# NeuroDiffGym/neurodiffeq

Hardware: AMD Instinct MI355X
Metric: collocation-points/sec (residual+bwd), 2D Laplace 65k pts, 1/2/4/8 GPU (higher is better)
Workload: dtype f32; 1 GPU; C2: Solver2D 2D Laplace, DirichletBVP2D, FCNN(2-32-32-1, tanh), Generator2D 256x256 = 65536 noisy-grid points per GPU per step, Adam(1e-3), run_train_epoch() with n_batches_train=1, n_batches_valid=0; points_per_gpu=65536, global_batch=65536, parallelism=dp1 (shard-by-batch, one all-reduce of [P+1] fp32 per step), allreduce=none (single process), inputs=pre-sampled in the reference's RNG order, resident in HBM

## Files before the change

__graft_entry__.py:

```python
import os
import sys

ROOT = os.path.dirname(os.path.abspath(__file__))
if ROOT not in sys.path:
    sys.path.insert(0, ROOT)


def build():
    from neurodiffeq_amd import _hipcc
    with _hipcc.deferred():
        built = _build_all()
    from neurodiffeq_amd import codegen
    for f in ([] if os.environ.get("NDQ_BUILD_NO_PRUNE") else os.listdir(codegen.JIT_DIR)):
        path = os.path.join(codegen.JIT_DIR, f)
        if path not in built and os.path.splitext(path)[0] + ".so" not in built:
            if os.path.isdir(path):
                import shutil
                shutil.rmtree(path, ignore_errors=True)
            else:
                os.remove(path)
    missing = [b for b in built if not os.path.exists(b)]
    assert not missing, f"build() did not produce {missing}"


# ... 34 lines not shown
        systems.append((name, nets, conds, pde, z.n_coords, None))
    pde, conds = zoo.spherical_solver_problem()
    systems.append(("spherical-default", [FCNN(3, 1)], conds, pde, 3, None))
    from neurodiffeq_amd import diff
    from neurodiffeq_amd.conditions import IVP
    losses = {}
    for name, kind in (("helmholtz_xy", "l1"), ("stokes_like", "l1"), ("stokes_like", "infinity"), ("pendulum", "infinity")):
        z = zoo.build(name)
        nets, conds, pde = z.product()
        systems.append((f"{name}/{kind}", nets, conds, pde, z.n_coords, None))
        losses[f"{name}/{kind}"] = kind
    systems.append(("default-ode/l1", [FCNN(1, 1)], [IVP(0.0, 1.0)], lambda u, t: [diff(u, t) + u], 1, None))
    losses["default-ode/l1"] = "l1"
    systems.append(("default-ode", [FCNN(1, 1)], [IVP(0.0, 1.0)], lambda u, t: [diff(u, t) + u], 1, None))
    from neurodiffeq_amd.solvers import sobolev_equations
    lv = lambda u, v, t: [diff(u, t) - (u - u * v), diff(v, t) - (u * v - v)]
    for semi in (False, True):
        systems.append((f"lotka-volterra/h1{' semi' if semi else ''}", [FCNN(1, 1), FCNN(1, 1)], [IVP(0.0, 1.5), IVP(0.0, 1.0)],
                        sobolev_equations(lv, 2, semi), 1, None))
    from neurodiffeq_amd.conditions import NoCondition
    systems.append(("helmholtz/h1", [FCNN(2, 1)], [NoCondition()],
                    sobolev_equations(lambda u, x, y: [diff(u, x, order=2) + diff(u, y, order=2) - u], 1, False), 2, None))
    for name in ("shell", "poisson3d", "hessian3d", "pendulum", "shape_48x2", "shape_32x3"):
        z = zoo.build(name)
        nets, conds, pde = z.product()
        systems.append((f"{name}/group", nets, conds, pde, z.n_coords, None))
    import warnings
    shared = FCNN(1, 2, hidden_units=(32, 32))
    sconds = [IVP(0.0, 1.5), IVP(0.0, 1.0)]
    with warnings.catch_warnings():
        warnings.simplefilter("ignore")
        sconds[0].set_impose_on(0)
        sconds[1].set_impose_on(1)
    systems.append(("shared-net", [shared, shared], sconds, lv, 1, None))
    from functools import partial
    from neurodiffeq_amd.networks import Resnet, Swish
    c4 = configs.make("c4", 8)
    systems.append(("c4/resnet", [Resnet(1, 25, hidden_units=(32, 32))], c4["conds"], configs.fused_equations(c4),
                    configs.n_coords(c4), configs.func_val(c4)))
    c2 = configs.make("c2", 8)
    systems.append(("c2/swish-trainable", [FCNN(2, 1, hidden_units=(32, 32), actv=partial(Swish, trainable=True))], c2["conds"],
                    configs.fused_equations(c2), configs.n_coords(c2), configs.func_val(c2)))
    c2n, c3n = configs.make("c2", 8), configs.make("c3", 8)
    systems.append(("c2/nolap", c2n["nets"], c2n["conds"], configs.fused_equations(c2n), 2, None))
    systems.append(("c2/columns", c2n["nets"], c2n["conds"],
                    lambda u, x, y: [diff(u, x), diff(u, y), diff(u, x, order=2), diff(u, y, order=2)], 2, None))
    systems.append(("c3/columns", c3n["nets"], c3n["conds"],
                    lambda u, x, y: [diff(u, x), diff(u, y), diff(u, x, order=2)], 2, None))
    for name in ("inv1", "inv2"):
        torch.manual_seed(0)
        icfg = configs.make_inverse(name)
        systems.append((name, icfg["nets"], icfg["conds"], icfg["pde"], 2 if name == "inv1" else 1, None))
    from tests import sampler_table_problems
    for axes in (2, 4):
        torch.manual_seed(0)
        tcfg = sampler_table_problems.bundle_problem(axes)
        systems.append((f"table-bundle-{axes}", tcfg["nets"], tcfg["conds"], tcfg["pde"], axes, None))
    csolver, ccfg = configs.make_custom_loss_solver(16)
    systems.append(("custom-loss", ccfg["nets"], ccfg["conds"], ccfg["pde"], 2, None))
    losses["custom-loss"] = lambda r, f, x: csolver.loss_fn(r, f, x) + csolver.additional_loss(r, f, x)
    metrics = {"custom-loss": list(csolver.metrics_fn.values())}
    for name, nets, conds, pde, nc, cfv in systems:
        os.environ.pop("NDQ_FUSE_GROUP", None)
        os.environ.pop("NDQ_NO_LAP", None)
        if name.endswith("/group"):
            os.environ["NDQ_FUSE_GROUP"] = "1"
        if name.endswith("/nolap"):
            os.environ["NDQ_NO_LAP"] = "1"
        program, descs = trace_system(nets, conds, pde, nc, compute_func_val=cfv, loss=losses.get(name, "l2"),
                                      metrics=metrics.get(name, ()))
        so = codegen.build(program)
        built.add(so)
        print("built", so, f"({name}: {len(program.symbols)} stream symbols, {len(program.order)} nodes)", flush=True)
        if codegen.can_fuse(program, descs):
            so = codegen.build_fused(program, descs[0])
            built.add(so)
            print("built", so, f"({name}: single-launch fused closure, {len(nets)} network(s))", flush=True)
            if name in ("c2", "pendulum", "advection", "helmholtz_xy", "sigmoid_mixed") and codegen.fuse_mode(program, descs) == "tile":
                so = codegen.build_fused(program, descs[0], threads=512)
                built.add(so)
                print("built", so, f"({name}: 8-wave build of the closure kernel)", flush=True)
    os.environ.pop("NDQ_FUSE_GROUP", None)
    os.environ.pop("NDQ_NO_LAP", None)
    f64_systems = []
    for name, size in (("c1", 8), ("c2", 8), ("c3", 8)):
        torch.manual_seed(0)
        cfg = configs.make(name, size)
        if name == "c3":
            cfg["nets"] = [FCNN(2, 1, hidden_units=(32, 32, 32))]
        f64_systems.append((name, cfg["nets"], cfg["conds"], configs.fused_equations(cfg), configs.n_coords(cfg), configs.func_val(cfg)))
    for name in ("pendulum", "helmholtz_xy", "stokes_like", "sigmoid_mixed", "kdv", "resnet_laplace", "swish_tr_laplace",
                 "aptx_tr_resnet", "shape_20x3", "mono_ode", "ensemble_lv", "shape_48x2", "shape_64x2"):
        z = zoo.build(name)
        nets, conds, pde = z.product()
        f64_systems.append((name, nets, conds, pde, z.n_coords, None))
    for name in ("c1", "c2", "c4", "w1", "w2", "w3", "w4", "w5", "w6", "w7", "w8", "w9", "w10", "w11", "w12", "w13", "w14", "w15",
                 "w16", "w17"):
        torch.manual_seed(0)
        cfg = configs.make(name, {"c1": 64, "c2": 16, "c4": 96}.get(name))
        f64_systems.append((name + "/golden", cfg["nets"], cfg["conds"], configs.fused_equations(cfg), configs.n_coords(cfg),
                            configs.func_val(cfg)))
    for name, nets, conds, pde, nc, cfv in f64_systems:
        for net in nets:
            net.double()
        program, descs = trace_system(nets, conds, pde, nc, compute_func_val=cfv, f64=True)
        so = codegen.build(program, f64=True)
        built.add(so)
        print("built", so, f"({name}: fp64 pointwise kernel)", flush=True)
        if codegen.can_fuse_f64(program, descs):
            so = codegen.build_fused(program, descs[0], f64=True)
            built.add(so)
            print("built", so, f"({name}: fp64 single-launch closure)", flush=True)
    from neurodiffeq_amd import autograd_ops
    for name in ("c1", "c2", "c3", "c4", "c5"):
        for net in configs.make(name, 8)["nets"][:1]:
            for order in (0, 1, 2):
                assert autograd_ops._spec_for(net, order) is not None, (name, order)
    for net in (FCNN(3, 2, hidden_units=(32, 32)), FCNN(1, 1), FCNN(3, 1)):
        for order in (0, 2):
            assert autograd_ops._spec_for(net, order) is not None
    for net in (FCNN(1, 1), FCNN(2, 1)):
        assert autograd_ops._spec_for(net, 3) is not None
    for L64 in (_lib.lib64(),):
        for sym in _lib.EXPORTS64:
            getattr(L64, sym)
    for d, act, n_out, order in ((2, 0, 3, 1), (3, 0, 1, 2), (1, 2, 1, 3), (2, 1, 1, 0), (1, 0, 1, 0), (2, 0, 1, 0)):
        assert codegen.ensure_mlp_kernels(autograd_ops._desc(d, order, 32, 2, act, n_out), f64=True), (d, act, n_out, order)
    for args in ((1, 1, 1, 32, 2, 1, 1, 0, 0, 1), (2, 1, 7, 32, 2, 0, 1, 0, 0, 15), (2, 1, 1, 32, 2, 0, 1, 0, 0, 1),
                 (2, 1, 5, 64, 3, 0, 1, 0, 0, 9), (1, 1, 1, 32, 2, 2, 2, 0, 0, 1), (3, 1, 22, 32, 2, 0, 1, 0, 0, 16)):
        assert codegen.ensure_mlp_kernels(_lib.MlpDesc(*args)), args
    assert codegen.ensure_mlp_kernels(autograd_ops._desc(2, 4, 32, 2, 0, 1)), "order-4 stream set of the autograd seam"
    from tests import test_gpu_parity as gp
    gp.ARCH.update(gp.ARCH_T4)
    try:
        for name in gp.ARCH_T4:
            assert codegen.ensure_mlp_kernels(gp._desc(name)), name
    finally:
        for name in gp.ARCH_T4:
            gp.ARCH.pop(name, None)
    from tests import test_gpu_netfamily as nf
    from tests import test_gpu_wide as wd
    ext_descs = [nf._desc(name) for name in nf.CASES]
    for shape in wd.SHAPES:
        ext_descs.append(wd.shape_desc(shape)[0])
    with _hipcc.deferred():
        for desc in ext_descs:
            if not L.ndq_mlp_supported(ctypes.byref(desc)) and codegen.mlp_ext_allowed(desc):
                codegen.build_mlp_ext(desc)
    for name in nf.CASES:
        assert codegen.ensure_mlp_kernels(nf._desc(name)), name
    from tests import test_gpu_wide as wd
    for shape in wd.SHAPES:
        assert codegen.ensure_mlp_kernels(wd.shape_desc(shape)[0]), shape
    built |= {ext._name for ext in codegen._MLP_EXT.values() if ext is not None}
    if os.path.isdir("/root/reference/neurodiffeq"):
        subprocess.run(["bash", os.path.join(ROOT, "oracle", "make_ref.sh")], check=True)
    return built


def smoke():
    import numpy as np
    import torch
    from oracle import autograd_ref as R
    from tests import configs
    assert torch.cuda.is_available(), "smoke() needs cuda:0"
    torch.cuda.set_device(0)
# ... 24 lines not shown
```

include/ndq.h:

```cpp
#ifndef NDQ_H
#define NDQ_H
#include <stddef.h>
#ifdef __cplusplus
extern "C" {
#endif

#define NDQ_EUNSUPPORTED (-1)
#define NDQ_EINVAL (-2)

#define NDQ_ACT_TANH 0
#define NDQ_ACT_SIN 1
#define NDQ_ACT_SIGMOID 2
#define NDQ_ACT_SWISH 3
#define NDQ_ACT_APTX 4
#define NDQ_ACT_ELU 5
#define NDQ_ACT_SOFTPLUS 6
#define NDQ_ACT_GELU 7

#define NDQ_MAX_HIDDEN 512
typedef struct ndq_mlp_desc {
  int d;
  int first;
  int mask2;
  int hidden;
// ... 44 lines not shown
                   float beta2, float eps, float weight_decay, int step, const float* loss_slots, int n_batches,
                   float* loss_hist, int hist_index, float* best_loss, int parity, float* best_flat, int write_scalars,
                   void* stream);

#define NDQ_SAMPLE_UNIFORM 0
#define NDQ_SAMPLE_GRID 1
#define NDQ_SAMPLE_SPHERICAL 2
typedef struct ndq_sampler_desc {
  int kind;
  int d;
  int n[3];
  float lo[3], hi[3];
  float noise_std[3];
  int radial;
} ndq_sampler_desc;
int ndq_sample(const ndq_sampler_desc* desc, unsigned long long seed, unsigned long long draw, unsigned stream_id,
               float* coords, int ldc, void* stream);

#define NDQ_TABLE_MAX_AXES 6
#define NDQ_AXIS_NORMAL 0
#define NDQ_AXIS_CHEB2_NOISY 1
typedef struct ndq_table_sampler_desc {
  int d;
  int n[NDQ_TABLE_MAX_AXES];
  int law[NDQ_TABLE_MAX_AXES];
  int abs_value;
  const float* mean[NDQ_TABLE_MAX_AXES];
  const float* std[NDQ_TABLE_MAX_AXES];
  float lo[NDQ_TABLE_MAX_AXES], hi[NDQ_TABLE_MAX_AXES];
} ndq_table_sampler_desc;
int ndq_sample_table(const ndq_table_sampler_desc* desc, unsigned long long seed, unsigned long long draw,
                     unsigned stream_id, float* coords , int ldc, void* stream);

#define NDQ_PLAN_MAX_LEAVES 8
#define NDQ_LEAF_SIMPLE 0
#define NDQ_LEAF_TABLE 1
#define NDQ_LEAF_DATA 2
#define NDQ_SEG_LEAF 0
#define NDQ_SEG_ENSEMBLE 1
#define NDQ_SEG_MESH 2
typedef struct ndq_plan_leaf {
  int kind;
  int row0;
  int rows;
  int n;
  union {
    ndq_sampler_desc simple;
    ndq_table_sampler_desc table;
    const float* data[NDQ_TABLE_MAX_AXES];
  } u;
} ndq_plan_leaf;
typedef struct ndq_plan_segment {
  int mode;
  int first, count;
  int offset, size;
} ndq_plan_segment;
typedef struct ndq_plan_sampler_desc {
  int d;
  int n_leaves;
  int n_segments;
  int reserved;
  ndq_plan_leaf leaf[NDQ_PLAN_MAX_LEAVES];
  ndq_plan_segment seg[NDQ_PLAN_MAX_LEAVES];
} ndq_plan_sampler_desc;
int ndq_sample_plan(const ndq_plan_sampler_desc* desc, unsigned long long seed, unsigned long long draw,
                    unsigned stream_id, float* coords , int ldc, void* stream);

#define NDQ_INDEX_NONE 0
#define NDQ_INDEX_PERMUTE 1
#define NDQ_INDEX_REPLACE 2
typedef struct ndq_plan_index_desc {
  int mode;
  int m;
  int batch;
  int reserved;
} ndq_plan_index_desc;
int ndq_sample_plan_indexed(const ndq_plan_sampler_desc* desc, const ndq_plan_index_desc* index, unsigned long long seed,
                            unsigned long long draw, unsigned stream_id, float* coords , int ldc, void* stream);

typedef int (*ndq_fused_launch_fn)(const float* coords, int ldc, int n, const float* params, float* partials,
                                   float* loss_partials, float* funcs, float* resid, int ldj, float seed, int train,
                                   void* stream);

typedef int (*ndq_allreduce_fn)(const void* sendbuf, void* recvbuf, size_t count, int dtype, int op, void* comm,
                                void* stream);

typedef struct ndq_fused_step {
  ndq_fused_launch_fn launch;
  int n, ldc, ldj, blocks, n_params;
  float seed;
  float* params;
  float* partials;
  float* loss_partials;
  float* grad;
  float* loss_slot;
  float* adam_m;
  float* adam_v;
  float lr, beta1, beta2, eps, weight_decay;
  float* loss_hist;
  float* best_loss;
  float* best_flat;
  ndq_allreduce_fn allreduce;
  void* comm;
  const struct ndq_sampler_desc* next_sampler;
  unsigned long long next_seed, next_draw;
  unsigned next_stream;
  float* next_coords;
  int next_ldc;
} ndq_fused_step;
int ndq_fused_step_run(const ndq_fused_step* s, const float* coords, int adam_step, int hist_index, int parity,
                       void* stream);

typedef int (*ndq_fused_launch_multi_fn)(const float* coords, int ldc, int n, const float* const* params,
                                         float* const* partials, float* loss_partials, float* funcs, float* resid,
                                         int ldj, float seed, int train, void* stream);
int ndq_fused_multi_step_run(const ndq_fused_step* steps, int n_nets, ndq_fused_launch_multi_fn launch,
                             const float* coords, int adam_step, int hist_index, int parity, void* stream);

typedef int (*ndq_fused_launch_tv_fn)(const float* coords, int ldc, int n, const float* const* params,
                                      float* const* partials, float* loss_partials, float seed,
                                      const float* valid_coords, int valid_ldc, int valid_n,
                                      float* valid_loss_partials, const void* pull, void* stream);
typedef int (*ndq_fused_launch_loop_fn)(const float* coords, int ldc, int n, float seed, const float* vcoords, int vldc,
                                        int vn, const void* loop, void* stream);
typedef struct ndq_fused_fit {
  ndq_fused_launch_tv_fn launch;
  int n_nets;
  ndq_fused_step net[4];
  const float* valid_coords;
  int valid_n, valid_ldc, valid_blocks;
  float valid_scale;
  float* valid_loss_partials;
  float* valid_hist;
  int track_best;
  int pull_ok;
  float* alt_params[4];
  float* alt_m[4];
  float* alt_v[4];
  float* alt_partials[4];
  float* alt_loss_partials;
  float* alt_valid_loss_partials;
  ndq_fused_launch_loop_fn launch_loop;
  int loop_ok;
} ndq_fused_fit;
int ndq_fused_fit_run(const ndq_fused_fit* f, int n_epochs, const float* const* train_coords, int adam_step,
                      int hist_index, int valid_index, int parity, void* stream);

typedef int (*ndq_pointwise_fn)(const float* coords, int ldc, int n, const float* const* jets,
                                float* const* gbar, int ldj, float* funcs, float* resid, float* loss_partials,
                                float seed_scale, void* stream);
typedef int (*ndq_pw_blocks_fn)(int n);
typedef void (*ndq_bind_theta_fn)(const float* theta, float* theta_partials);

typedef struct ndq64_mlp_kernels {
  ndq_mlp_desc desc;
  int n_streams, n_params;
  int bwd_waves;
  int lds_bytes;
  int (*fwd)(const double* coords, int ldc, int n, const double* params, double* jets, int ldj, void* stream);
  int (*bwd)(const double* coords, int ldc, int n, const double* params, const double* gbar, int ldj, double* partials,
             int blocks, void* stream);
} ndq64_mlp_kernels;
int ndq64_mlp_register(const ndq64_mlp_kernels* kernels);
int ndq64_mlp_supported(const ndq_mlp_desc* desc);
int ndq64_mlp_num_streams(const ndq_mlp_desc* desc);
int ndq64_mlp_num_params(const ndq_mlp_desc* desc);
int ndq64_mlp_bwd_blocks(const ndq_mlp_desc* desc, int n);
int ndq64_mlp_jet_fwd(const ndq_mlp_desc* desc, const double* coords, int ldc, int n, const double* params, double* jets,
                      int ldj, void* stream);
int ndq64_mlp_jet_bwd(const ndq_mlp_desc* desc, const double* coords, int ldc, int n, const double* params,
                      const double* gbar, int ldj, double* partials, void* stream);
int ndq64_reduce_partials(const double* partials, int nparts, int len, double* out, int accumulate, double scale,
                          void* stream);
int ndq64_adam_step(double* params, const double* grad, double* exp_avg, double* exp_avg_sq, int len, double lr,
                    double beta1, double beta2, double eps, double weight_decay, int step, void* stream);

int ndq64_epoch_tail(double* params, const double* grad, double* exp_avg, double* exp_avg_sq, int len, double lr,
                     double beta1, double beta2, double eps, double weight_decay, int step, const double* loss_slots,
                     int n_batches, double* loss_hist, int hist_index, double* best_loss, int parity, double* best_flat,
                     int write_scalars, void* stream);

int ndq_oneshot_create(int rank, int world_size, int max_len, void** ctx, unsigned char* handle64);
int ndq_oneshot_connect(void* ctx, const unsigned char* handles);
int ndq_oneshot_allreduce(const void* send, void* recv, size_t count, int dtype, int op, void* ctx, void* stream);
int ndq_oneshot_status(void* ctx);
int ndq_oneshot_destroy(void* ctx);

#ifdef __cplusplus
}
#endif
#endif
// ... 1 lines not shown
```

neurodiffeq_amd/_lib.py:

```python
import ctypes
import os

from . import _build

NDQ_ACT_TANH, NDQ_ACT_SIN, NDQ_ACT_SIGMOID, NDQ_ACT_SWISH, NDQ_ACT_APTX = 0, 1, 2, 3, 4
NDQ_ACT_ELU, NDQ_ACT_SOFTPLUS, NDQ_ACT_GELU = 5, 6, 7


class MlpDesc(ctypes.Structure):
    _fields_ = [("d", ctypes.c_int), ("first", ctypes.c_int), ("mask2", ctypes.c_int), ("hidden", ctypes.c_int),
                ("layers", ctypes.c_int), ("act", ctypes.c_int), ("n_out", ctypes.c_int), ("lap", ctypes.c_int),
                ("skip", ctypes.c_int), ("mask3", ctypes.c_int), ("actp", ctypes.c_int), ("widths", ctypes.c_int), ("mono", ctypes.c_int),
                ("mask4", ctypes.c_int)]

    def key(self):
        return (self.d, self.first, self.mask2, self.hidden, self.layers, self.act, self.n_out, self.lap, self.skip,
                self.mask3, self.actp, self.widths, self.mono, self.mask4)


NDQ_SAMPLE_UNIFORM, NDQ_SAMPLE_GRID, NDQ_SAMPLE_SPHERICAL = 0, 1, 2


class SamplerDesc(ctypes.Structure):
    _fields_ = [("kind", ctypes.c_int), ("d", ctypes.c_int), ("n", ctypes.c_int * 3), ("lo", ctypes.c_float * 3),
                ("hi", ctypes.c_float * 3), ("noise_std", ctypes.c_float * 3), ("radial", ctypes.c_int)]


NDQ_TABLE_MAX_AXES = 6
NDQ_AXIS_NORMAL, NDQ_AXIS_CHEB2_NOISY = 0, 1


class TableSamplerDesc(ctypes.Structure):
    _fields_ = [("d", ctypes.c_int), ("n", ctypes.c_int * 6), ("law", ctypes.c_int * 6), ("abs_value", ctypes.c_int),
                ("mean", ctypes.c_void_p * 6), ("std", ctypes.c_void_p * 6), ("lo", ctypes.c_float * 6),
                ("hi", ctypes.c_float * 6)]


NDQ_PLAN_MAX_LEAVES = 8
NDQ_LEAF_SIMPLE, NDQ_LEAF_TABLE, NDQ_LEAF_DATA = 0, 1, 2
NDQ_SEG_LEAF, NDQ_SEG_ENSEMBLE, NDQ_SEG_MESH = 0, 1, 2
NDQ_INDEX_NONE, NDQ_INDEX_PERMUTE, NDQ_INDEX_REPLACE = 0, 1, 2


class _PlanLaw(ctypes.Union):
    _fields_ = [("simple", SamplerDesc), ("table", TableSamplerDesc), ("data", ctypes.c_void_p * 6)]


class PlanLeaf(ctypes.Structure):
    _fields_ = [("kind", ctypes.c_int), ("row0", ctypes.c_int), ("rows", ctypes.c_int), ("n", ctypes.c_int), ("u", _PlanLaw)]


class PlanSegment(ctypes.Structure):
    _fields_ = [("mode", ctypes.c_int), ("first", ctypes.c_int), ("count", ctypes.c_int), ("offset", ctypes.c_int),
                ("size", ctypes.c_int)]


class PlanSamplerDesc(ctypes.Structure):
    _fields_ = [("d", ctypes.c_int), ("n_leaves", ctypes.c_int), ("n_segments", ctypes.c_int), ("reserved", ctypes.c_int),
                ("leaf", PlanLeaf * 8), ("seg", PlanSegment * 8)]


class PlanIndexDesc(ctypes.Structure):
    _fields_ = [("mode", ctypes.c_int), ("m", ctypes.c_int), ("batch", ctypes.c_int), ("reserved", ctypes.c_int)]


FUSED_LAUNCH_FN = ctypes.CFUNCTYPE(ctypes.c_int, ctypes.c_void_p, ctypes.c_int, ctypes.c_int, ctypes.c_void_p,
                                   ctypes.c_void_p, ctypes.c_void_p, ctypes.c_void_p, ctypes.c_void_p, ctypes.c_int,
                                   ctypes.c_float, ctypes.c_int, ctypes.c_void_p)


class FusedStep(ctypes.Structure):
    _fields_ = [("launch", ctypes.c_void_p),
                ("n", ctypes.c_int), ("ldc", ctypes.c_int), ("ldj", ctypes.c_int), ("blocks", ctypes.c_int),
                ("n_params", ctypes.c_int), ("seed", ctypes.c_float),
                ("params", ctypes.c_void_p), ("partials", ctypes.c_void_p), ("loss_partials", ctypes.c_void_p),
                ("grad", ctypes.c_void_p), ("loss_slot", ctypes.c_void_p), ("adam_m", ctypes.c_void_p),
                ("adam_v", ctypes.c_void_p),
                ("lr", ctypes.c_float), ("beta1", ctypes.c_float), ("beta2", ctypes.c_float), ("eps", ctypes.c_float),
                ("weight_decay", ctypes.c_float),
                ("loss_hist", ctypes.c_void_p), ("best_loss", ctypes.c_void_p), ("best_flat", ctypes.c_void_p),
                ("allreduce", ctypes.c_void_p), ("comm", ctypes.c_void_p),
                ("next_sampler", ctypes.c_void_p), ("next_seed", ctypes.c_ulonglong), ("next_draw", ctypes.c_ulonglong),
                ("next_stream", ctypes.c_uint), ("next_coords", ctypes.c_void_p), ("next_ldc", ctypes.c_int)]


class FusedFit(ctypes.Structure):
    _fields_ = [("launch", ctypes.c_void_p), ("n_nets", ctypes.c_int), ("net", FusedStep * 4),
                ("valid_coords", ctypes.c_void_p), ("valid_n", ctypes.c_int), ("valid_ldc", ctypes.c_int),
                ("valid_blocks", ctypes.c_int), ("valid_scale", ctypes.c_float),
                ("valid_loss_partials", ctypes.c_void_p), ("valid_hist", ctypes.c_void_p), ("track_best", ctypes.c_int),
                ("pull_ok", ctypes.c_int), ("alt_params", ctypes.c_void_p * 4), ("alt_m", ctypes.c_void_p * 4),
                ("alt_v", ctypes.c_void_p * 4), ("alt_partials", ctypes.c_void_p * 4),
                ("alt_loss_partials", ctypes.c_void_p), ("alt_valid_loss_partials", ctypes.c_void_p),
                ("launch_loop", ctypes.c_void_p), ("loop_ok", ctypes.c_int)]


class NdqError(RuntimeError):
    pass


_LIB = None


def lib():
    global _LIB
    if _LIB is not None:
        return _LIB
    path = _build.LIB
    if _build.is_stale():
        try:
            _build.build_lib()
        except Exception as e:
            if not os.path.exists(path):
                raise NdqError(f"libndq.so is missing and could not be built: {e}") from e
    L = ctypes.CDLL(path)
    vp, ci, cf = ctypes.c_void_p, ctypes.c_int, ctypes.c_float
    dp = ctypes.POINTER(MlpDesc)
    L.ndq_mlp_supported.argtypes = [dp]
    L.ndq_mlp_num_streams.argtypes = [dp]
    L.ndq_mlp_num_params.argtypes = [dp]
    L.ndq_mlp_bwd_blocks.argtypes = [dp, ci]
    L.ndq_mlp_jet_fwd.argtypes = [dp, vp, ci, ci, vp, vp, ci, vp]
    L.ndq_mlp_jet_bwd.argtypes = [dp, vp, ci, ci, vp, vp, ci, vp, vp]
    L.ndq_reduce_partials.argtypes = [vp, ci, ci, vp, ci, cf, vp]
    L.ndq_adam_step.argtypes = [vp, vp, vp, vp, ci, cf, cf, cf, cf, cf, ci, vp]
    L.ndq_reduce_grad_loss.argtypes = [vp, ci, ci, vp, ci, vp, ci, vp, cf, vp]
    L.ndq_epoch_tail.argtypes = [vp, vp, vp, vp, ci, cf, cf, cf, cf, cf, ci, vp, ci, vp, ci, vp, ci, vp, ci, vp]
    L.ndq_fused_step_run.argtypes = [ctypes.POINTER(FusedStep), vp, ci, ci, ci, vp]
    L.ndq_fused_multi_step_run.argtypes = [ctypes.POINTER(FusedStep), ci, vp, vp, ci, ci, ci, vp]
    L.ndq_fused_fit_run.argtypes = [ctypes.POINTER(FusedFit), ci, vp, ci, ci, ci, ci, vp]
    L.ndq_mlp_register.argtypes = [vp]
    L.ndq_sample.argtypes = [ctypes.POINTER(SamplerDesc), ctypes.c_ulonglong, ctypes.c_ulonglong, ctypes.c_uint, vp, ci, vp]
    L.ndq_sample_table.argtypes = [ctypes.POINTER(TableSamplerDesc), ctypes.c_ulonglong, ctypes.c_ulonglong, ctypes.c_uint, vp, ci,
                                   vp]
    L.ndq_sample_plan.argtypes = [ctypes.POINTER(PlanSamplerDesc), ctypes.c_ulonglong, ctypes.c_ulonglong, ctypes.c_uint, vp, ci, vp]
    L.ndq_sample_plan_indexed.argtypes = [ctypes.POINTER(PlanSamplerDesc), ctypes.POINTER(PlanIndexDesc), ctypes.c_ulonglong,
                                          ctypes.c_ulonglong, ctypes.c_uint, vp, ci, vp]
    L.ndq_oneshot_create.argtypes = [ci, ci, ci, ctypes.POINTER(vp), ctypes.c_char_p]
    L.ndq_oneshot_connect.argtypes = [vp, ctypes.c_char_p]
    L.ndq_oneshot_allreduce.argtypes = [vp, vp, ctypes.c_size_t, ci, ci, vp, vp]
    L.ndq_oneshot_status.argtypes = [vp]
    L.ndq_oneshot_destroy.argtypes = [vp]
    for name in ("ndq_mlp_supported", "ndq_mlp_num_streams", "ndq_mlp_num_params", "ndq_mlp_bwd_blocks",
                 "ndq_mlp_jet_fwd", "ndq_mlp_jet_bwd", "ndq_reduce_partials", "ndq_adam_step", "ndq_reduce_grad_loss",
                 "ndq_epoch_tail", "ndq_fused_step_run", "ndq_sample", "ndq_sample_table", "ndq_sample_plan", "ndq_sample_plan_indexed", "ndq_mlp_register",
                 "ndq_fused_multi_step_run", "ndq_fused_fit_run", "ndq_oneshot_create", "ndq_oneshot_connect",
                 "ndq_oneshot_allreduce", "ndq_oneshot_status",
                 "ndq_oneshot_destroy"):
        getattr(L, name).restype = ci
    _LIB = L
    return L


_LIB64 = None


def lib64():
    global _LIB64
    if _LIB64 is not None:
        return _LIB64
    if _build.is_stale64():
        try:
            _build.build_lib64()
        except Exception as e:
            if not os.path.exists(_build.LIB64):
                raise NdqError(f"libndq64.so is missing and could not be built: {e}") from e
# ... 35 lines not shown
```

neurodiffeq_amd/codegen.py:

```python
import ctypes
import hashlib
import os
import re

from .symbolic import Graph, TraceUnsupported

HERE = os.path.dirname(os.path.abspath(__file__))
JIT_DIR = os.path.join(HERE, "_jit")
from . import _hipcc


def _extra_flags():
    return os.environ.get("NDQ_JIT_FLAGS", "").split()


def pair_list(d):
    return [(a, b) for a in range(d) for b in range(a, d)]


def triple_list(d):
    return [(a, b, c) for a in range(d) for b in range(a, d) for c in range(b, d)]


CLOSURE_PRODUCTS = ("#ifndef NDQ_HBAR_NPROD\n#define NDQ_HBAR_NPROD 4\n#endif\n"
# ... 34 lines not shown
            self.mask2 |= 1 << pair_list(self.d).index(loc)
        if len(loc) == 3:
            self.mask3 |= 1 << triple_list(self.d).index(loc)
            for pair in ((loc[0], loc[1]), (loc[0], loc[2]), (loc[1], loc[2])):
                self.mask2 |= 1 << pair_list(self.d).index(pair)
        if len(loc) == 4:
            if self.d > 3:
                raise TraceUnsupported("fourth-order derivatives of a network with more than three inputs are outside the fused path")
            self.mask4 |= 1 << quad_list(self.d).index(loc)
            for i in range(4):
                tri = tuple(loc[j] for j in range(4) if j != i)
                self.mask3 |= 1 << triple_list(self.d).index(tri)
                for j in range(i + 1, 4):
                    self.mask2 |= 1 << pair_list(self.d).index((loc[i], loc[j]))
        if len(loc) > 4:
            raise TraceUnsupported("derivatives of network outputs beyond fourth order are outside the fused path")

    @property
    def n_streams(self):
        return (1 + self.first * self.d + (1 if self.lap else bin(self.mask2).count("1")) + bin(self.mask3).count("1")
                + bin(self.mask4).count("1"))

    def slot(self, mi):
        if mi and mi[0] == "L":
            return 1 + self.d
        assert not (self.lap and len(mi) == 2)
        loc = tuple(sorted(self.deps.index(c) for c in mi))
        if len(loc) == 0:
            return 0
        if len(loc) == 1:
            return 1 + loc[0]
        if len(loc) == 4:
            k = quad_list(self.d).index(loc)
            assert (self.mask4 >> k) & 1 and not self.lap
            return 1 + self.d + bin(self.mask2).count("1") + bin(self.mask3).count("1") + bin(self.mask4 & ((1 << k) - 1)).count("1")
        if len(loc) == 3:
            k = triple_list(self.d).index(loc)
            assert (self.mask3 >> k) & 1 and not self.lap
            return 1 + self.d + bin(self.mask2).count("1") + bin(self.mask3 & ((1 << k) - 1)).count("1")
        k = pair_list(self.d).index(loc)
        assert (self.mask2 >> k) & 1
        return 1 + self.d + bin(self.mask2 & ((1 << k) - 1)).count("1")


def _lit(v):
    if v != v or v in (float("inf"), float("-inf")):
        raise ValueError("non-finite constant in traced expression")
    s = repr(float(v))
    if "." not in s and "e" not in s and "n" not in s:
        s += ".0"
    return s + "f"


def _powi_expr(x, n):
    if n == 0:
        return "1.0f"
    if n == 1:
        return x
    if n <= 8:
        return "(" + "*".join([x] * n) + ")"
    return f"powf({x}, {float(n)}f)"


_UN_FWD = {
    "neg": "-{a}", "sin": "sinf({a})", "cos": "cosf({a})", "tan": "tanf({a})", "exp": "expf({a})",
    "log": "logf({a})", "tanh": "tanhf({a})", "sqrt": "sqrtf({a})", "abs": "fabsf({a})", "sinh": "sinhf({a})",
    "cosh": "coshf({a})", "sigmoid": "(1.0f/(1.0f+expf(-{a})))", "recip": "(1.0f/{a})",
    "sign": "(({a}>0.0f)-({a}<0.0f))",
    "log1p": "log1pf({a})", "expm1": "expm1f({a})", "erf": "erff({a})", "atan": "atanf({a})",
    "floor": "floorf({a})", "ceil": "ceilf({a})", "round": "rintf({a})", "trunc": "truncf({a})",
    "detach": "{a}",
}
_UN_ADJ = {
    "neg": "-{b}", "sin": "{b}*cosf({a})", "cos": "-{b}*sinf({a})", "tan": "{b}*(1.0f+{v}*{v})",
    "exp": "{b}*{v}", "log": "{b}/{a}", "tanh": "{b}*(1.0f-{v}*{v})", "sqrt": "{b}/(2.0f*{v})",
    "abs": "{b}*(({a}>0.0f)-({a}<0.0f))", "sinh": "{b}*coshf({a})", "cosh": "{b}*sinhf({a})",
    "sigmoid": "{b}*{v}*(1.0f-{v})", "recip": "-{b}*{v}*{v}", "sign": None,
    "log1p": "{b}/(1.0f+{a})", "expm1": "{b}*({v}+1.0f)", "erf": "{b}*1.1283791670955126f*expf(-{a}*{a})",
    "atan": "{b}/(1.0f+{a}*{a})",
    "floor": None, "ceil": None, "round": None, "trunc": None, "detach": None,
}


def _closure_host(K, threads, points, slots, kern, kern_tv, lds, kern_loop=None, lds_loop=None):
    return f"""struct Closure {{
  using Cfg = CFG;
  using Pw = PW;
  using Args = ndq::{'FusedArgs' if K == 1 else 'FusedMultiArgs'};
  static constexpr int K = {K}, THREADS = {threads}, POINTS = {points}, SLOTS = {slots};
  static constexpr auto train = &{kern('true')};
  static constexpr auto eval = &{kern('false')};
  static constexpr auto tv = &{kern_tv};
  static constexpr auto loop = {'&' + kern_loop if kern_loop else 'nullptr'};
  static constexpr size_t LDS_TRAIN = {lds('true')}, LDS_EVAL = {lds('false')}, LDS_LOOP = {lds_loop or 0};
}};
}}  // namespace
#include "ndq_closure_host.h"
"""


class PointwiseProgram:

    LOSS_KINDS = ("l2", "l1", "infinity", "custom")

    def __init__(self, graph: Graph, residuals, funcs, n_nets, widen=None, allow_lap=None, unify=None, loss="l2",
                 loss_term=None):
        assert loss in self.LOSS_KINDS and (loss == "custom") == (loss_term is not None)
        self.loss = loss
        self.g = graph
        self.residuals = list(residuals)
        self.funcs = list(funcs)
        self.loss_term = loss_term
        if allow_lap is not None:
            extra = [loss_term] if loss_term is not None else []
            merged = self._merge_laplacian(self.residuals + extra, self.funcs, n_nets, allow_lap)
            self.residuals = merged[:len(self.residuals)]
            if extra:
                self.loss_term = merged[-1]
        self.n_nets = n_nets
        self.site_net = list(getattr(graph, "site_net", None) or range(n_nets))
        self.n_sites = len(self.site_net)
        self.n_coords = graph.n_coords
        self.n_data = len(getattr(graph, "data", ()))
        self.n_theta = len(getattr(graph, "params", ()))
        self.order = graph.reachable(self.residuals + self.funcs + ([self.loss_term] if self.loss_term is not None else []))
        self.streams = {}
        for k in range(self.n_sites):
            deps = graph.net_deps.get(k)
            if deps is None:
                continue
            self.streams[k] = NetStreams(deps, graph.net_nout[k])
        self.symbols = []
        for i in self.order:
            n = graph.nodes[i]
            if n[0] == "net":
                self.streams[n[1]].need(n[3])
                self.symbols.append(i)
        if unify is not None:
            unify(self.streams)
        if widen is not None:
            for k, st in self.streams.items():
                widen(k, st)
        self.source = self._emit()
        self.key = hashlib.sha1((self.source + _build_tag()).encode()).hexdigest()[:16]

    def _merge_laplacian(self, residuals, funcs, n_nets, allow_lap):
        g = self.g
        order = g.reachable(list(residuals) + list(funcs))
        second = {}
        third = set()
        for i in order:
            n = g.nodes[i]
            if n[0] == "net" and len(n[3]) == 2 and n[3][0] != "L":
                second.setdefault(n[1], []).append(i)
            if n[0] == "net" and len(n[3]) >= 3 and n[3][0] != "L":
                third.add(n[1])
        for k in third:
            second.pop(k, None)
        func_set = set(g.reachable(list(funcs)))
        out = list(residuals)
        for k, leaves in second.items():
            mis = [g.nodes[i][3] for i in leaves]
            if any(a != b for a, b in mis) or len(leaves) < 2:
                continue
            if any(i in func_set for i in leaves):
                continue
            by_out = {}
            for i in leaves:
                by_out.setdefault(g.nodes[i][2], []).append(i)
            coords = sorted({mi[0] for mi in mis})
            if any(sorted(g.nodes[i][3][0] for i in ls) != coords for ls in by_out.values()):
                continue
            leafset = set(leaves)
            ok = True
            for r in out:
                for o, ls in by_out.items():
                    ds = [g.diff(r, ("n", i)) for i in ls]
# ... 136 lines not shown
            i = g._ids.get(("param", j))
            L.append(f"  g[{nsym + j}] = {'b%d' % i if (i is not None and i in terms and i in res_set) else '0.0f'};")
        return "\n".join(L)

    def point_fn_source(self):
        nc = self.n_coords
        body = self._emit_point_fn()
        neq = len(self.residuals)
        if self.loss == "custom":
            term = f"r[{neq}]"
        elif self.loss == "l2":
            term = " + ".join(f"r[{e}]*r[{e}]" for e in range(neq)) or "0.0f"
        elif self.loss == "l1":
            term = " + ".join(f"fabsf(r[{e}])" for e in range(neq)) or "0.0f"
        else:
            term = "0.0f"
            for e in range(neq):
                term = f"fmaxf({term}, fabsf(r[{e}]))"
        nd, nt = self.n_data, self.n_theta
        return f"""// c: {nc} coordinate(s) | {nd} per-point data value(s) | {nt} trainable scalar(s) of the equations;  g: adjoints of the
// {len(self.symbols)} stream symbol(s) | of the {nt} trainable scalar(s)
NDQ_PW_INLINE void ndq_pw_point(const float* c, const float* s, float seed, int want_adj, float* r, float* f, float* g) {{
{chr(10).join(f"  const float c{i} = c[{i}];" for i in range(nc))}
{chr(10).join(f"  const float d{j} = c[{nc + j}];" for j in range(nd))}
{chr(10).join(f"  const float t{j} = c[{nc + nd + j}];" for j in range(nt))}
{chr(10).join(f"  const float c{i} = {_lit(v)};   // virtual coordinate (boundary value)" for i, v in sorted(self.g.vcoords.items()))}
{body}
}}
// per-point loss term ({self.loss}); the host averages it: seed = 1 / (N * n_eq) for l2 / l1, 1 / N for infinity
NDQ_PW_INLINE float ndq_pw_loss(const float* r) {{ return {term}; }}
"""

    @property
    def loss_norm(self):
        return 1 if self.loss in ("infinity", "custom") else max(len(self.residuals), 1)

    @property
    def n_r(self):
        return max(len(self.residuals) + (1 if self.loss == "custom" else 0), 1)

    def fused_source(self, desc, f64=False):
        if f64:
            return "#define NDQ_F64 1\n" + source_f64(self._fused_source(desc, True))
        return self._fused_source(desc, False)

    def _fused_source(self, desc, f64):
        K = self.n_nets
        mode = fuse_mode(self, {k: desc for k in range(K)})
        assert mode is not None and not (f64 and (mode != "tile" or K != 1))
        if mode in ("group", "wide"):
            return self._group_source(desc, wide=(mode == "wide"))
        ns = self.streams[0].n_streams
        nsym = max(len(self.symbols), 1)
        jet = (lambda k, loc: f"jets[{loc}]") if K == 1 else (lambda k, loc: f"jets[{k}][{loc}]")
        gj = (lambda k, loc: f"gj[{loc}]") if K == 1 else (lambda k, loc: f"gj[{k}][{loc}]")
        loads, stores = [], []
        used = {}
        for idx, i in enumerate(self.symbols):
            k, loc = self.sym_location(i)
            used[(k, loc)] = idx
            loads.append(f"    s[{idx}] = {jet(k, loc)};")
        for k in range(K):
            for loc in range(ns):
                stores.append(f"    {gj(k, loc)} = {'g[%d]' % used[(k, loc)] if (k, loc) in used else '0.0f'};")
        header = "ndq_mlp.h"
        neq, nf = len(self.residuals), len(self.funcs)
        jets_t = "const float (&jets)[CFG::NS]" if K == 1 else f"const float (&jets)[{K}][CFG::NS]"
        gj_t = "float (&gj)[CFG::NS]" if K == 1 else f"float (&gj)[{K}][CFG::NS]"
        kern = (lambda train: f"ndq::fused_closure_kernel<CFG, PW, {train}>") if K == 1 else \
            (lambda train: f"ndq::fused_multi_closure_kernel<CFG, {K}, PW, {train}>")
        lds = (lambda train: f"ndq::fused_lds_bytes<CFG>({train})") if K == 1 else \
            (lambda train: f"(ndq::fused_multi_lds_bytes<CFG, {K}>({train}))")
        threads = "CFG::BWD_THREADS" if K == 1 else f"ndq::multi_threads<{K}>()"
        tiles_per_block = "CFG::BWD_THREADS / 64" if K == 1 else f"ndq::multi_group<{K}>()"
        kern_tv = "ndq::fused_closure_tv_kernel<CFG, PW>" if K == 1 else f"ndq::fused_multi_closure_tv_kernel<CFG, {K}, PW>"
        if f64:
            kern_loop = lds_loop = None
        elif K == 1:
            kern_loop, lds_loop = "ndq::fused_closure_loop_kernel<CFG, PW>", "ndq::fused_loop_lds_bytes<CFG>()"
        elif K == 2:
            kern_loop, lds_loop = f"ndq::fused_multi_closure_loop_kernel<CFG, {K}, PW>", f"(ndq::fused_multi_loop_lds_bytes<CFG, {K}>())"
        else:
            kern_loop = lds_loop = None
        host = _closure_host(K, threads, 16, tiles_per_block, kern, kern_tv, lds, kern_loop, lds_loop)
        wg_tr = f"#ifndef NDQ_WG_TR\n#define NDQ_WG_TR 1\n#endif\n#define NDQ_WG_TR_K {K}\n" + CLOSURE_PRODUCTS
        return f"""// GENERATED by neurodiffeq_amd/codegen.py -- single-launch closure kernel (forward streams + pointwise stage +
// reverse pass) of one PDE system with {K} network(s), gfx950.
{wg_tr}#include "{header}"
#define NDQ_PW_INLINE __device__ __forceinline__
#ifndef NDQ_MAX_BLOCKS
#define NDQ_MAX_BLOCKS 256     // closure workgroups per launch (one per CU; experiments: 512 = two 8-wave workgroups per CU)
#endif
{self.point_fn_source()}
namespace {{
using CFG = {mlp_cfg(desc, 1)};
struct PW {{
  // ND per-point data columns (rows D .. D + ND of the coordinate block), NT trainable scalars of the equations
  static constexpr int NEQ = {neq}, NF = {nf}, NR = {self.n_r}, ND = {self.n_data}, NT = {self.n_theta};
  static __device__ __forceinline__ float loss(const float* r) {{ return ndq_pw_loss(r); }}
  // xe: the point's ND data values, then the NT scalars;  gth (want_adj): per-point adjoints of the scalars
  static __device__ __forceinline__ void apply(const float (&x)[CFG::D], const float* xe, {jets_t}, float seed,
                                               int want_adj, float (&r)[{self.n_r}], float (&f)[{max(nf, 1)}],
                                               {gj_t}, float* gth) {{
    float c[CFG::D + ND + NT], s[{nsym}], g[{nsym} + NT];
#pragma unroll
    for (int d = 0; d < CFG::D; ++d) c[d] = x[d];
#pragma unroll
    for (int j = 0; j < ND + NT; ++j) c[CFG::D + j] = xe[j];
{chr(10).join(loads)}
    ndq_pw_point(c, s, seed, want_adj, r, f, g);
{chr(10).join(stores)}
#pragma unroll
    for (int j = 0; j < NT; ++j) gth[j] = g[{len(self.symbols)} + j];
  }}
}};
{host}"""

    def _group_source(self, desc, wide=False):
        st = self.streams[0]
        width = st.n_streams * st.n_out
        gw = 1 if st.n_out == 1 else (st.n_out + 15) // 16 * 16
        if wide:
            gw = st.n_out
        row = lambda loc: (loc // st.n_out) * gw + loc % st.n_out
        nsym = max(len(self.symbols), 1)
        used = {}
        loads = []
        for idx, i in enumerate(self.symbols):
            k, loc = self.sym_location(i)
            used[loc] = idx
            loads.append(f"    s[{idx}] = srow[{row(loc)}];")
        stores = [f"    grow[{row(loc)}] = {'g[%d]' % used[loc] if loc in used else '0.0f'};" for loc in range(width)]
        deps = list(st.deps)
        dep_fn = " : ".join(f"d == {d} ? {c}" for d, c in enumerate(deps)) + " : 0"
        header = "ndq_mlp.h"
        neq, nf = len(self.residuals), len(self.funcs)
        kern = lambda train: f"ndq::fused_group_closure_kernel<CFG, PW, {train}>"
        lds = lambda train: f"ndq::group_lds_bytes<CFG>({train})"
        kern_tv = "ndq::fused_group_closure_tv_kernel<CFG, PW>"
        cfg_t, points = mlp_cfg(desc, desc.n_out), "16 * ndq::group_tiles<CFG>()"
        if wide:
            header = "ndq_wide.h"
            kern = lambda train: f"ndq::wide_closure_kernel<CFG, PW, {train}>"
            lds = lambda train: "(ndq::wide_closure_lds_bytes<CFG, PW>())"
            kern_tv = "ndq::wide_closure_tv_kernel<CFG, PW>"
            cfg_t, points = wide_cfg(desc), 16
        host = _closure_host(1, "CFG::BWD_THREADS", points, "CFG::BWD_THREADS / 64", kern, kern_tv, lds)
        return f"""// GENERATED by neurodiffeq_amd/codegen.py -- grouped single-launch closure kernel (forward streams -> LDS exchange ->
// per-point stage, one point per lane -> reverse pass) of one PDE system, gfx950.
{CLOSURE_PRODUCTS}#include "{header}"
#define NDQ_PW_INLINE __device__ __forceinline__
#ifndef NDQ_MAX_BLOCKS
#define NDQ_MAX_BLOCKS 256     // closure workgroups per launch (one per CU; experiments: 512 = two 8-wave workgroups per CU)
#endif
{self.point_fn_source()}
namespace {{
using CFG = {cfg_t};
static_assert(CFG::NS * CFG::NOUT == {width}, "stream layout of the traced program and of the kernel disagree");
struct PW {{
  // NC rows of the coordinate block per point: the batch coordinates, then ND data columns; NT trainable scalars
  static constexpr int NEQ = {neq}, NF = {nf}, ND = {self.n_data}, NT = {self.n_theta}, NC = {self.n_coords} + ND, NR = {self.n_r};
  static constexpr int dep(int d) {{ return {dep_fn}; }}     // batch coordinate fed to network input d
  static __device__ __forceinline__ float loss(const float* r) {{ return ndq_pw_loss(r); }}
  static __device__ __forceinline__ void apply(const float (&cc)[NC], const float* th, const float* srow, float seed, int want_adj,
                                               float (&r)[{self.n_r}], float (&f)[{max(nf, 1)}], float* grow, float* gth) {{
    float c[NC + NT], s[{nsym}], g[{nsym} + NT];
#pragma unroll
# ... 132 lines not shown
    a.jets[k] = jets[k];
    a.gbar[k] = gbar ? gbar[k] : nullptr;
  }}
  a.funcs = funcs; a.resid = resid; a.loss_partials = loss_partials;
  a.n = n; a.ldc = ldc; a.ldj = ldj; a.want_adj = gbar ? 1 : 0; a.seed = seed_scale;
  hipLaunchKernelGGL(ndq_pw_kernel, dim3((n + 255) / 256), dim3(256), 0, static_cast<hipStream_t>(stream), a);
  return (int)hipGetLastError();
}}
#endif
"""
        return src

    def bytes_per_point(self, train=True, write_resid=False, write_funcs=False):
        b = 4 * self.n_coords + 4 * len(self.symbols)
        if train:
            b += 4 * sum(st.n_streams * st.n_out for st in self.streams.values())
        if write_resid:
            b += 4 * len(self.residuals)
        if write_funcs:
            b += 4 * len(self.funcs)
        return b


class PointwiseKernel:
    def __init__(self, so_path, f64=False):
        self.path = so_path
        self.lib = ctypes.CDLL(so_path)
        self.lib.ndq_pw_launch.restype = ctypes.c_int
        self.lib.ndq_pw_launch.argtypes = [ctypes.c_void_p, ctypes.c_int, ctypes.c_int, ctypes.c_void_p, ctypes.c_void_p,
                                           ctypes.c_int, ctypes.c_void_p, ctypes.c_void_p, ctypes.c_void_p,
                                           ctypes.c_double if f64 else ctypes.c_float, ctypes.c_void_p]
        self.lib.ndq_pw_blocks.restype = ctypes.c_int
        self.lib.ndq_pw_blocks.argtypes = [ctypes.c_int]

    def blocks(self, n):
        return self.lib.ndq_pw_blocks(n)


def so_path_for(program: PointwiseProgram, f64=False):
    return os.path.join(JIT_DIR, f"pw{'64' if f64 else ''}_{program.key}.so")


_F64_FUNCS = re.compile(r"\b(pow|sin|cos|tan|exp|log|tanh|sqrt|fabs|sinh|cosh|fmax|log1p|expm1|erf|atan|atan2|floor|ceil|rint|trunc)f\(")
_F64_LITERAL = re.compile(r"(?<![\w.])((?:\d+\.\d*|\.\d+|\d+)(?:[eE][-+]?\d+)?)f\b")


def source_f64(source):
    out = re.sub(r"\bfloat\b", "double", source)
    out = _F64_FUNCS.sub(lambda m: m.group(1) + "(", out)
    return _F64_LITERAL.sub(lambda m: m.group(1), out)


def build(program: PointwiseProgram, force=False, f64=False):
    os.makedirs(JIT_DIR, exist_ok=True)
    so = so_path_for(program, f64)
    src = so[:-3] + ".hip"
    if os.path.exists(so) and not force:
        return so
    with open(src, "w") as fh:
        fh.write(source_f64(program.source) if f64 else program.source)
    try:
        _hipcc.compile_shared(src, so, defer=True)
    except RuntimeError as e:
        raise RuntimeError(f"hipcc failed for generated pointwise kernel {src}:\n{str(e)[-4000:]}") from e
    return so


def load(program: PointwiseProgram, f64=False):
    return PointwiseKernel(build(program, f64=f64), f64)


class FusedKernel:
    def __init__(self, so_path, f64=False):
        self.path = so_path
        self.lib = ctypes.CDLL(so_path)
        vp, ci, cf = ctypes.c_void_p, ctypes.c_int, (ctypes.c_double if f64 else ctypes.c_float)
        self.lib.ndq_fused_launch.restype = ci
        self.lib.ndq_fused_launch.argtypes = [vp, ci, ci, vp, vp, vp, vp, vp, ci, cf, ci, vp]
        self.lib.ndq_fused_launch_multi.restype = ci
        self.lib.ndq_fused_launch_multi.argtypes = [vp, ci, ci, vp, vp, vp, vp, vp, ci, cf, ci, vp]
        self.lib.ndq_fused_launch_tv.restype = ci
        self.lib.ndq_fused_launch_tv.argtypes = [vp, ci, ci, vp, vp, vp, cf, vp, ci, ci, vp, vp, vp]
        self.lib.ndq_fused_pull_ok.restype = ci
        self.lib.ndq_fused_launch_loop.restype = ci
        self.lib.ndq_fused_launch_loop.argtypes = [vp, ci, ci, cf, vp, ci, ci, vp, vp]
        self.lib.ndq_fused_loop_ok.restype = ci
        self.lib.ndq_fused_bind_theta.restype = None
        self.lib.ndq_fused_bind_theta.argtypes = [vp, vp]
        self.lib.ndq_fused_blocks.restype = ci
        self.lib.ndq_fused_blocks.argtypes = [ci]
        self.lib.ndq_fused_num_params.restype = ci
        self.lib.ndq_fused_num_nets.restype = ci
        self.lib.ndq_fused_threads.restype = ci
        self.threads = self.lib.ndq_fused_threads()
        self.lib.ndq_fused_lds_bytes.restype = ctypes.c_ulong
        self.n_nets = self.lib.ndq_fused_num_nets()

    def blocks(self, n):
        return self.lib.ndq_fused_blocks(n)


def _cache_key(source):
    text = source.replace(HERE, "<neurodiffeq_amd>")
    return hashlib.sha1((text + _header_digest() + " ".join(_extra_flags()) + _build_tag()).encode()).hexdigest()[:16]


def _build_tag():
    return _hipcc.FIXUP_VERSION if _hipcc.fixup_enabled() else "no-fixup"


def _header_digest():
    h = hashlib.sha1()
    for name in ("csrc/ndq_mlp.h", "csrc/ndq_tail.h", "csrc/ndq_launch.h", "csrc/ndq_wide.h", "csrc/ndq_deep.h", "csrc/ndq_closure_host.h",
                 "../include/ndq.h"):
        with open(os.path.join(HERE, name), "rb") as fh:
            h.update(fh.read())
    return h.hexdigest()


_MLP_EXT = {}


MAX_INPUTS = 6
MAX_LAYERS = 8


def mlp_ext_allowed(desc):
    if os.environ.get("NDQ_JIT_MLP", "1") == "0":
        return False
    npair = desc.d * (desc.d + 1) // 2
    diag = 0
    for a in range(desc.d):
        diag |= 1 << pair_list(desc.d).index((a, a))
    if desc.mask3:
        if desc.lap or desc.d > 4 or desc.act not in (0, 1, 2, 5, 6, 7) or desc.mask3 >> len(triple_list(desc.d)):
            return False
        for k, (a, b, c) in enumerate(triple_list(desc.d)):
            if (desc.mask3 >> k) & 1 and not all((desc.mask2 >> pair_list(desc.d).index(p)) & 1
                                                   for p in ((a, b), (a, c), (b, c))):
                return False
    if desc.mask4:
        if (desc.lap or desc.d > 3 or desc.act not in (0, 1, 2) or desc.actp or desc.mono or is_wide(desc)
                or desc.mask4 >> len(quad_list(desc.d))):
            return False
        for k, q in enumerate(quad_list(desc.d)):
            if (desc.mask4 >> k) & 1:
                for i in range(4):
                    tri = tuple(q[j] for j in range(4) if j != i)
                    if not (desc.mask3 >> triple_list(desc.d).index(tri)) & 1:
                        return False
                    for j in range(i + 1, 4):
                        if not (desc.mask2 >> pair_list(desc.d).index((q[i], q[j]))) & 1:
                            return False
    if desc.widths:
        bits, most = (10, 3) if is_wide(desc) else (8, 4)
        ws = [(desc.widths >> (bits * l)) & ((1 << bits) - 1) for l in range(most)]
        if (desc.widths >> (bits * most)) or desc.layers > most or any(w for w in ws[desc.layers:]) or min(ws[:desc.layers]) < 1 \
                or max(ws[:desc.layers]) != desc.hidden or (is_wide(desc) and desc.layers < 2):
            return False
    if desc.mono and (not 0 < desc.mono < 256 or desc.mask3 or desc.skip or desc.hidden > 48):
        return False
    if is_wide(desc) and (desc.skip or desc.actp or desc.mono or desc.n_out > 16):
        return False
    return (1 <= desc.d <= MAX_INPUTS and 1 <= desc.hidden <= MAX_HIDDEN and 1 <= desc.layers <= (4 if desc.widths else MAX_LAYERS)
            and desc.act in (0, 1, 2, 3, 4, 5, 6, 7) and 1 <= desc.n_out <= 64 and desc.first in (0, 1)
            and 0 <= desc.mask2 < (1 << npair) and (desc.first == 1 or desc.mask2 == 0)
# ... 171 lines not shown
```

neurodiffeq_amd/csrc/ndq_api.hip:

```cpp
#include <cstdlib>
#include <vector>
#include "ndq_launch.h"
#include "ndq_sample.h"
#include "ndq_oneshot.h"
#include "ndq_tail.h"

extern "C" int ndq_oneshot_allreduce(const void* send, void* recv, size_t count, int dtype, int op, void* comm, void* stream);

namespace ndq {

#ifndef NDQ_CFG_TABLE
#define NDQ_CFG_TABLE(X)      \
  X(1, 0, 0, 2, 2, ACT_SIN, 1, 0)   \
  X(1, 1, 0, 2, 2, ACT_SIN, 1, 0)   \
  X(1, 1, 1, 2, 2, ACT_SIN, 1, 0)   \
  X(1, 0, 0, 2, 2, ACT_TANH, 1, 0)  \
  X(1, 1, 0, 2, 2, ACT_TANH, 1, 0)  \
  X(1, 1, 1, 2, 2, ACT_TANH, 1, 0)  \
  X(2, 0, 0, 2, 2, ACT_TANH, 1, 0)  \
  X(2, 1, 0, 2, 2, ACT_TANH, 1, 0)  \
  X(2, 1, 1, 2, 2, ACT_TANH, 1, 0)  \
  X(2, 1, 5, 2, 2, ACT_TANH, 1, 0)  \
  X(2, 1, 7, 2, 2, ACT_TANH, 1, 0)  \
  X(2, 0, 0, 4, 3, ACT_TANH, 1, 0)  \
// ... 77 lines not shown
      const int r = rg + 16 * j;
      v[j] = part[(size_t)(r < nparts ? r : nparts - 1) * len + cc];
    }
  }
  __device__ __forceinline__ float finish(const float* __restrict__ part, int nparts, int len, int col, int rg) const {
    float x[16];
#pragma unroll
    for (int j = 0; j < 16; ++j) x[j] = v[j];
    asm volatile("" : "+v"(x[0]), "+v"(x[1]), "+v"(x[2]), "+v"(x[3]), "+v"(x[4]), "+v"(x[5]), "+v"(x[6]), "+v"(x[7]), "+v"(x[8]),
                      "+v"(x[9]), "+v"(x[10]), "+v"(x[11]), "+v"(x[12]), "+v"(x[13]), "+v"(x[14]), "+v"(x[15]));
#pragma unroll
    for (int j = 0; j < 16; ++j) x[j] = (rg + 16 * j < nparts && col < len) ? x[j] : 0.f;
    float s0 = 0.f, s1 = 0.f, s2 = 0.f, s3 = 0.f;
#pragma unroll
    for (int it = 0; it < 4; ++it) {
      if (rg + 64 * it + 48 < nparts) { s0 += x[4 * it]; s1 += x[4 * it + 1]; s2 += x[4 * it + 2]; s3 += x[4 * it + 3]; }
      else { s0 += x[4 * it]; s0 += x[4 * it + 1]; s0 += x[4 * it + 2]; s0 += x[4 * it + 3]; }
    }
    if (nparts > 256 && col < len) {
      int r = rg + 256;
      for (; r + 48 < nparts; r += 64) {
        s0 += part[(size_t)r * len + col];
        s1 += part[(size_t)(r + 16) * len + col];
        s2 += part[(size_t)(r + 32) * len + col];
        s3 += part[(size_t)(r + 48) * len + col];
      }
      for (; r < nparts; r += 16) s0 += part[(size_t)r * len + col];
    }
    return (s0 + s1) + (s2 + s3);
  }
};

__device__ __forceinline__ float column_sum_1024(const float* __restrict__ part, int nparts, int len, int col, int rg,
                                                 float* sm ) {
  ColumnRows rows;
  rows.issue(part, nparts, len, col, rg);
  sm[rg * 64 + (threadIdx.x & 63)] = rows.finish(part, nparts, len, col, rg);
  __syncthreads();
  float s = 0.f;
  if (rg == 0) {
#pragma unroll
    for (int g = 0; g < 16; ++g) s += sm[g * 64 + (threadIdx.x & 63)];
  }
  return s;
}

__device__ __forceinline__ float block_sum_1024(const float* __restrict__ v, int n, float* sm16) {
  float x = 0.f;
  for (int r = threadIdx.x; r < n; r += 1024) x += v[r];
  for (int off = 32; off > 0; off >>= 1) x += __shfl_down(x, off);
  if ((threadIdx.x & 63) == 0) sm16[threadIdx.x >> 6] = x;
  __syncthreads();
  float s = 0.f;
  if (threadIdx.x == 0)
    for (int w = 0; w < 16; ++w) s += sm16[w];
  return s;
}

__global__ __launch_bounds__(1024) void reduce_grad_loss_kernel(Reduce2Args a) {
  __shared__ float sm[16 * 64];
  if (blockIdx.x + 1 < gridDim.x) {
    const int c = threadIdx.x & 63, rg = threadIdx.x >> 6;
    const int i = blockIdx.x * 64 + c;
    const float s = column_sum_1024(a.part, a.nparts, a.len, i, rg, sm);
    if (rg == 0 && i < a.len) a.out[i] = a.accumulate ? a.out[i] + s : s;
  } else {
    const float s = block_sum_1024(a.lpart, a.nlparts, sm);
    if (threadIdx.x == 0) *a.lout = s * a.lscale;
  }
}

using TailArgs = ndq::TailArgsT<float>;

struct ValidArgs {
  const float* part; int nparts; float scale; float* hist; int index;
  int best_on_valid;
};
struct ReduceTailArgs {
  Reduce2Args r;
  TailArgs t;
  int tail_blocks;
  ndq::SampleArgs smp;
  ValidArgs v;
};
#ifndef NDQ_TAIL_COLS
#define NDQ_TAIL_COLS 64
#endif
template <int TC>
__device__ __forceinline__ void reduce_tail_body(const ReduceTailArgs& a) {
  constexpr int TT = TC * 16, WAVES = TT / 64;
  __shared__ float sm[16 * TC];
  __shared__ float smw[16];
  __shared__ float smv[16];
  const int tid = threadIdx.x, c = tid % TC, rg = tid / TC, lane = tid & 63, wave = tid >> 6;
  const int i = blockIdx.x * TC + c;
  const bool col = i < a.r.len;
  const bool has_valid = a.v.part != nullptr;
  const bool has_train = a.r.nparts > 0;
  ColumnRows rows;
  if (has_train) rows.issue(a.r.part, a.r.nparts, a.r.len, i, rg);
  const float lp0 = tid < a.r.nlparts ? a.r.lpart[tid] : 0.f;
  const float vp0 = has_valid && tid < a.v.nparts ? a.v.part[tid] : 0.f;
  const bool upd = (rg == 0) && col;
  const float* p_in = a.t.p_in ? a.t.p_in : a.t.p;
  const float* m_in = a.t.m_in ? a.t.m_in : a.t.m;
  const float* v_in = a.t.v_in ? a.t.v_in : a.t.v;
  float pi = 0.f, m0 = 0.f, v0 = 0.f;
  if (upd) {
    pi = p_in[i];
    if (has_train || a.t.p_in) { m0 = m_in[i]; v0 = v_in[i]; }
  }
  const float best = a.t.best_loss[a.t.parity];
  float lp = lp0, vp = vp0;
  for (int r = tid + TT; r < a.r.nlparts; r += TT) lp += a.r.lpart[r];
  if (has_valid)
    for (int r = tid + TT; r < a.v.nparts; r += TT) vp += a.v.part[r];
  const float colsum = has_train ? rows.finish(a.r.part, a.r.nparts, a.r.len, i, rg) : 0.f;
  for (int off = 32; off > 0; off >>= 1) lp += __shfl_down(lp, off);
  if (has_valid)
    for (int off = 32; off > 0; off >>= 1) vp += __shfl_down(vp, off);
  if (lane == 0) { smw[wave] = lp; smv[wave] = vp; }
  sm[rg * TC + c] = colsum;
  __syncthreads();
  float loss = 0.f, vloss = 0.f;
#pragma unroll
  for (int w = 0; w < WAVES; ++w) loss += smw[w];
  loss *= a.r.lscale;
  if (has_valid) {
#pragma unroll
    for (int w = 0; w < WAVES; ++w) vloss += smv[w];
    vloss *= a.v.scale;
  }
  const bool on_valid = has_valid && a.v.best_on_valid != 0;
  const float cmp = on_valid ? vloss : loss;
  const bool better = (a.t.best_flat != nullptr) && (on_valid || has_train) && (cmp < best);
  if (upd) {
    if (better) a.t.best_flat[i] = pi;
    if (has_train) {
      float g = 0.f;
#pragma unroll
      for (int k = 0; k < 16; ++k) g += sm[k * TC + c];
      a.r.out[i] = g;
      float pn, mi, vi;
      ndq::adam_value(a.t.adam, pi, g, m0, v0, pn, mi, vi);
      a.t.m[i] = mi;
      a.t.v[i] = vi;
      a.t.p[i] = pn;
    } else if (a.t.p_in) {
      a.t.p[i] = pi; a.t.m[i] = m0; a.t.v[i] = v0;
    }
  }
  if (blockIdx.x == 0 && tid == 0 && a.t.write_scalars) {
    if (has_train) {
      *a.r.lout = loss;
      a.t.loss_hist[a.t.hist_index] = loss;
    }
    if (has_valid) a.v.hist[a.v.index] = vloss;
    a.t.best_loss[a.t.parity ^ 1] = better ? cmp : best;
  }
}
__global__ __launch_bounds__(1024) void reduce_tail_kernel(ReduceTailArgs a) {
  if ((int)blockIdx.x >= a.tail_blocks) {
    ndq::sample_point_store(a.smp, ((int)blockIdx.x - a.tail_blocks) * 1024 + (int)threadIdx.x);
    return;
  }
  reduce_tail_body<64>(a);
}

__global__ __launch_bounds__(1024) void reduce_tail_dp_kernel(ReduceTailArgs a, ndq::OneshotDev c, unsigned step) {
  __shared__ float sm[16 * 64];
  __shared__ float smw[16];
  __shared__ float sloss;
  __shared__ int timed_out;
  if (threadIdx.x == 0) timed_out = 0;
  const int tid = threadIdx.x, col = tid & 63, rg = tid >> 6, blk = blockIdx.x;
  const int i = blk * 64 + col;
  const bool incol = i < a.r.len;
  ColumnRows rows;
  rows.issue(a.r.part, a.r.nparts, a.r.len, i, rg);
  const float lp0 = tid < a.r.nlparts ? a.r.lpart[tid] : 0.f;
  const bool upd = (rg == 0) && incol;
  float pi = 0.f, m0 = 0.f, v0 = 0.f;
  if (upd) { pi = a.t.p[i]; m0 = a.t.m[i]; v0 = a.t.v[i]; }
  const float best = a.t.best_loss[a.t.parity];
  float lp = lp0;
  for (int r = tid + 1024; r < a.r.nlparts; r += 1024) lp += a.r.lpart[r];
  const float colsum = rows.finish(a.r.part, a.r.nparts, a.r.len, i, rg);
  for (int off = 32; off > 0; off >>= 1) lp += __shfl_down(lp, off);
  if (col == 0) smw[rg] = lp;
  sm[rg * 64 + col] = colsum;
  __syncthreads();
  const int parity = step & 1u;
  const size_t slot = ((size_t)parity * c.world + c.rank) * c.max_len + (size_t)blk * 65;
  if (rg == 0) {
    float g = 0.f;
#pragma unroll
    for (int k = 0; k < 16; ++k) g += sm[k * 64 + col];
    for (int q = 0; q < c.world; ++q)
      __hip_atomic_store(c.inbox[q] + slot + col, incol ? g : 0.f, __ATOMIC_RELAXED, __HIP_MEMORY_SCOPE_SYSTEM);
    if (col == 0) {
      float loss = 0.f;
#pragma unroll
      for (int w = 0; w < 16; ++w) loss += smw[w];
      loss *= a.r.lscale;
      for (int q = 0; q < c.world; ++q)
        __hip_atomic_store(c.inbox[q] + slot + 64, loss, __ATOMIC_RELAXED, __HIP_MEMORY_SCOPE_SYSTEM);
    }
  }
  __threadfence_system();
  __syncthreads();
  if (tid < c.world) {
    unsigned* f = c.flags[tid] + ((size_t)parity * c.world + c.rank) * c.max_blocks + blk;
    __hip_atomic_store(f, step, __ATOMIC_RELEASE, __HIP_MEMORY_SCOPE_SYSTEM);
    const unsigned* mine = c.flags[c.rank] + ((size_t)parity * c.world + tid) * c.max_blocks + blk;
    if (!ndq::oneshot_wait(mine, step, c.spin_limit, c.status)) timed_out = 1;
  }
  __syncthreads();
  const bool bad = timed_out != 0;
  const float* inbox = c.inbox[c.rank] + (size_t)parity * c.world * c.max_len + (size_t)blk * 65;
  if (tid == 0) {
    float loss = 0.f;
    for (int q = 0; q < c.world; ++q)
      loss += __hip_atomic_load(inbox + (size_t)q * c.max_len + 64, __ATOMIC_RELAXED, __HIP_MEMORY_SCOPE_SYSTEM);
    sloss = bad ? __builtin_nanf("") : loss;
  }
  __syncthreads();
  const float loss = sloss;
  const bool better = (a.t.best_flat != nullptr) && (loss < best);
  if (upd && !bad) {
    float g = 0.f;
// ... 41 lines not shown
extern "C" {

int ndq_mlp_supported(const ndq_mlp_desc* desc) { return find(desc) ? 1 : 0; }

int ndq_mlp_register(const ndq_mlp_kernels* k) {
  if (!k || !k->fwd || !k->bwd || k->desc.hidden < 1 || k->desc.hidden > NDQ_MAX_HIDDEN || k->n_streams < 1 || k->n_params < 1 || k->bwd_waves < 1 ||
      k->lds_bytes > 160 * 1024)
    return NDQ_EINVAL;
  if (!find(&k->desc)) g_registered.push_back(k);
  return 0;
}

int ndq_mlp_num_streams(const ndq_mlp_desc* desc) {
  const ndq_mlp_kernels* e = find(desc);
  return e ? e->n_streams : NDQ_EUNSUPPORTED;
}

int ndq_mlp_num_params(const ndq_mlp_desc* desc) {
  const ndq_mlp_kernels* e = find(desc);
  return e ? e->n_params : NDQ_EUNSUPPORTED;
}

int ndq_mlp_bwd_blocks(const ndq_mlp_desc* desc, int n) {
  const ndq_mlp_kernels* e = find(desc);
  if (!e) return NDQ_EUNSUPPORTED;
  if (n <= 0) return NDQ_EINVAL;
  return bwd_blocks(e->bwd_waves, n);
}

int ndq_mlp_jet_fwd(const ndq_mlp_desc* desc, const float* coords, int ldc, int n, const float* params, float* jets,
                    int ldj, void* stream) {
  const ndq_mlp_kernels* e = find(desc);
  if (!e) return NDQ_EUNSUPPORTED;
  if (!coords || !params || !jets || n <= 0 || ldc < n || ldj < n) return NDQ_EINVAL;
  return e->fwd(coords, ldc, n, params, jets, ldj, stream);
}

int ndq_mlp_jet_bwd(const ndq_mlp_desc* desc, const float* coords, int ldc, int n, const float* params,
                    const float* gbar, int ldj, float* partials, void* stream) {
  const ndq_mlp_kernels* e = find(desc);
  if (!e) return NDQ_EUNSUPPORTED;
  if (!coords || !params || !gbar || !partials || n <= 0 || ldc < n || ldj < n) return NDQ_EINVAL;
  return e->bwd(coords, ldc, n, params, gbar, ldj, partials, bwd_blocks(e->bwd_waves, n), stream);
}

int ndq_reduce_partials(const float* partials, int nparts, int len, float* out, int accumulate, float scale,
                        void* stream) {
  if (!partials || !out || nparts <= 0 || len <= 0) return NDQ_EINVAL;
  hipLaunchKernelGGL(reduce_partials_kernel, dim3((len + 255) / 256), dim3(256), 0, static_cast<hipStream_t>(stream),
                     partials, nparts, len, out, accumulate, scale);
  return (int)hipGetLastError();
}

int ndq_reduce_grad_loss(const float* partials, int nparts, int len, float* out, int accumulate,
                         const float* loss_partials, int n_loss_parts, float* loss_out, float loss_scale, void* stream) {
  if (!partials || !out || !loss_partials || !loss_out || nparts <= 0 || len <= 0 || n_loss_parts <= 0) return NDQ_EINVAL;
  Reduce2Args a{partials, nparts, len, out, accumulate, loss_partials, n_loss_parts, loss_out, loss_scale};
  hipLaunchKernelGGL(reduce_grad_loss_kernel, dim3((len + 63) / 64 + 1), dim3(1024), 0, static_cast<hipStream_t>(stream), a);
  return (int)hipGetLastError();
}

int ndq_epoch_tail(float* params, const float* grad, float* exp_avg, float* exp_avg_sq, int len, float lr, float beta1,
                   float beta2, float eps, float weight_decay, int step, const float* loss_slots, int n_batches,
                   float* loss_hist, int hist_index, float* best_loss, int parity, float* best_flat, int write_scalars,
                   void* stream) {
  const bool adam = exp_avg != nullptr;
  if (!params || len <= 0 || !loss_slots || n_batches <= 0 || !loss_hist || !best_loss || hist_index < 0 ||
      (parity != 0 && parity != 1) || (adam && (!grad || !exp_avg_sq || step <= 0)))
    return NDQ_EINVAL;
  TailArgs a{};
  a.p = params; a.g = grad; a.m = exp_avg; a.v = exp_avg_sq; a.len = len;
  a.adam = adam_consts(lr, beta1, beta2, eps, weight_decay, adam ? step : 0);
  a.loss_slots = loss_slots; a.nb = n_batches; a.loss_hist = loss_hist; a.hist_index = hist_index;
  a.best_loss = best_loss; a.parity = parity; a.best_flat = best_flat; a.write_scalars = write_scalars;
  hipLaunchKernelGGL(epoch_tail_kernel<float>, dim3((len + 255) / 256), dim3(256), 0, static_cast<hipStream_t>(stream), a);
  return (int)hipGetLastError();
}

}

static ReduceTailArgs reduce_tail_args(const ndq_fused_step& s, const ndq_fused_step& s0, const float* part, const float* lpart,
                                       int nparts, int adam_step, int hist_index, int parity, int write_scalars,
                                       float* best_flat, const ValidArgs& v = ValidArgs{}, const float* p_in = nullptr,
                                       const float* m_in = nullptr, const float* v_in = nullptr) {
  ReduceTailArgs a{};
  a.r = Reduce2Args{part, nparts, s.n_params, s.grad, 0, lpart, nparts, s.loss_slot, s0.seed};
  a.t.p = s.params; a.t.g = s.grad; a.t.m = s.adam_m; a.t.v = s.adam_v; a.t.len = s.n_params;
  a.t.adam = adam_consts(s.lr, s.beta1, s.beta2, s.eps, s.weight_decay, adam_step);
  a.t.p_in = p_in; a.t.m_in = m_in; a.t.v_in = v_in;
  a.t.loss_slots = s.loss_slot; a.t.nb = 1; a.t.loss_hist = s0.loss_hist; a.t.hist_index = hist_index;
  a.t.best_loss = s0.best_loss; a.t.parity = parity; a.t.best_flat = best_flat; a.t.write_scalars = write_scalars;
  a.tail_blocks = 0x7fffffff;
  a.v = v;
  return a;
}

extern "C" {

int ndq_fused_step_run(const ndq_fused_step* s, const float* coords, int adam_step, int hist_index, int parity,
                       void* stream) {
  if (!s || !s->launch || !coords) return NDQ_EINVAL;
  int rc = s->launch(coords, s->ldc, s->n, s->params, s->partials, s->loss_partials, nullptr, nullptr, s->ldj, s->seed,
                     1, stream);
  if (rc) return rc;
  if (!s->adam_m)
    return ndq_reduce_grad_loss(s->partials, s->blocks, s->n_params, s->grad, 0, s->loss_partials, s->blocks,
                                s->loss_slot, s->seed, stream);
  if (adam_step <= 0 || hist_index < 0 || (parity != 0 && parity != 1) || !s->loss_hist || !s->best_loss) return NDQ_EINVAL;
  const bool oneshot = s->allreduce == reinterpret_cast<ndq_allreduce_fn>(&ndq_oneshot_allreduce) && s->comm &&
                       ((s->n_params + 63) / 64) * 65 <= static_cast<ndq::Oneshot*>(s->comm)->dev.max_len &&
                       (s->n_params + 63) / 64 <= static_cast<ndq::Oneshot*>(s->comm)->dev.max_blocks;
  if (s->allreduce && !oneshot) {
    if (s->loss_slot != s->grad + s->n_params) return NDQ_EINVAL;
    rc = ndq_reduce_grad_loss(s->partials, s->blocks, s->n_params, s->grad, 0, s->loss_partials, s->blocks, s->loss_slot,
                              s->seed, stream);
    if (rc) return rc;
    rc = s->allreduce(s->grad, s->grad, (size_t)s->n_params + 1,  7,  0, s->comm, stream);
    if (rc) return 1000 + rc;
    return ndq_epoch_tail(s->params, s->grad, s->adam_m, s->adam_v, s->n_params, s->lr, s->beta1, s->beta2, s->eps,
                          s->weight_decay, adam_step, s->loss_slot, 1, s->loss_hist, hist_index, s->best_loss, parity,
                          s->best_flat, 1, stream);
  }
  ReduceTailArgs a = reduce_tail_args(*s, *s, s->partials, s->loss_partials, s->blocks, adam_step, hist_index, parity, 1,
                                      s->best_flat);
  int blocks = (s->n_params + 63) / 64;
  if (oneshot) {
    ndq::Oneshot* c = static_cast<ndq::Oneshot*>(s->comm);
    const unsigned step = ++c->step;
    hipLaunchKernelGGL(reduce_tail_dp_kernel, dim3(blocks), dim3(1024), 0, static_cast<hipStream_t>(stream), a, c->dev, step);
    return (int)hipGetLastError();
  }
  a.tail_blocks = blocks;
  if (s->next_sampler) {
    rc = ndq::fill_sample_args(a.smp, s->next_sampler, s->next_seed, s->next_draw, s->next_stream, s->next_coords,
                               s->next_ldc);
    if (rc) return rc;
    blocks += (a.smp.total + 1023) / 1024;
  }
  hipLaunchKernelGGL(reduce_tail_kernel, dim3(blocks), dim3(1024), 0, static_cast<hipStream_t>(stream), a);
  return (int)hipGetLastError();
}

int ndq_fused_multi_step_run(const ndq_fused_step* steps, int n_nets, ndq_fused_launch_multi_fn launch,
                             const float* coords, int adam_step, int hist_index, int parity, void* stream) {
  if (!steps || !launch || !coords || n_nets < 1 || n_nets > 4 || adam_step <= 0 || hist_index < 0 ||
      (parity != 0 && parity != 1))
    return NDQ_EINVAL;
  const ndq_fused_step& s0 = steps[0];
  if (!s0.loss_hist || !s0.best_loss || !s0.loss_partials) return NDQ_EINVAL;
  const float* params[4];
  float* partials[4];
  for (int k = 0; k < n_nets; ++k) {
    if (!steps[k].params || !steps[k].partials || !steps[k].grad || !steps[k].adam_m || !steps[k].adam_v ||
        !steps[k].loss_slot)
      return NDQ_EINVAL;
    params[k] = steps[k].params;
    partials[k] = steps[k].partials;
  }
  int rc = launch(coords, s0.ldc, s0.n, params, partials, s0.loss_partials, nullptr, nullptr, s0.ldj, s0.seed, 1, stream);
  if (rc) return rc;
  ReduceTailMultiArgs a{};
  int max_params = 0;
  for (int k = 0; k < n_nets; ++k) {
    a.net[k] = reduce_tail_args(steps[k], s0, steps[k].partials, s0.loss_partials, s0.blocks, adam_step, hist_index, parity,
                                k == 0 ? 1 : 0, steps[k].best_flat);
    if (steps[k].n_params > max_params) max_params = steps[k].n_params;
  }
  return launch_tail_multi(a, max_params, n_nets, s0.blocks, stream);
}

}

struct FitCall {
  const ndq_fused_fit* f;
  int n_epochs; const float* const* train_coords;
  int adam_step, hist_index, valid_index;
  void* stream;
  bool valid;
  int max_params, max_lparts;
  float* P[2][4]; float* M[2][4]; float* V[2][4]; float* PART[2][4]; float* LP[2]; float* VP[2];
};

static bool fit_tracks(const ndq_fused_fit* f, bool with_train, bool with_valid) {
  return (f->track_best == 1 && with_train) || (f->track_best == 2 && with_valid);
}

static int fit_tail(const FitCall& c, int set, bool with_train, bool with_valid, int adam_step, int hist_index, int vindex,
                    int parity) {
  const ndq_fused_fit* f = c.f;
  const ndq_fused_step& s0 = f->net[0];
  ValidArgs v{};
  if (with_valid) v = ValidArgs{c.VP[set], f->valid_blocks, f->valid_scale, f->valid_hist, vindex, f->track_best == 2 ? 1 : 0};
  const bool track = fit_tracks(f, with_train, with_valid);
  ReduceTailMultiArgs a{};
  for (int k = 0; k < f->n_nets; ++k) {
    const ndq_fused_step& s = f->net[k];
    a.net[k] = reduce_tail_args(s, s0, c.PART[set][k], c.LP[set], with_train ? s0.blocks : 0, with_train ? adam_step : 0,
                                hist_index, parity, k == 0 ? 1 : 0, track ? s.best_flat : nullptr, v,
                                set ? c.P[set][k] : nullptr, set ? c.M[set][k] : nullptr, set ? c.V[set][k] : nullptr);
  }
  return launch_tail_multi(a, c.max_params, f->n_nets, c.max_lparts, c.stream);
}

static int fit_two_launch(const FitCall& c, int parity) {
  const ndq_fused_fit* f = c.f;
  const ndq_fused_step& s0 = f->net[0];
  for (int e = 0; e < c.n_epochs; ++e, parity ^= 1) {
    if (!c.train_coords[e]) return NDQ_EINVAL;
    const bool with_valid = c.valid && e > 0;
    int rc = f->launch(c.train_coords[e], s0.ldc, s0.n, c.P[0], c.PART[0], c.LP[0], s0.seed,
                       with_valid ? f->valid_coords : nullptr, f->valid_ldc, with_valid ? f->valid_n : 0, c.VP[0], nullptr,
                       c.stream);
    if (rc) return rc;
    rc = fit_tail(c, 0, true, with_valid, c.adam_step + e, c.hist_index + e, c.valid_index + e - 1, parity);
    if (rc) return rc;
  }
  if (!c.valid) return 0;
  int rc = f->launch(nullptr, 0, 0, c.P[0], nullptr, nullptr, 0.f, f->valid_coords, f->valid_ldc, f->valid_n, c.VP[0], nullptr,
                     c.stream);
  if (rc) return rc;
  return fit_tail(c, 0, false, true, 0, c.hist_index + c.n_epochs, c.valid_index + (c.n_epochs > 0 ? c.n_epochs - 1 : 0), parity);
}

struct Finishes { int adam_step, hist_index, valid_index; bool with_valid; };
static Finishes launch_finishes(const FitCall& c, int e) {
  const int j = e - 1;
  return {c.adam_step + j, c.hist_index + j, c.valid_index + j - 1, c.valid && j >= 1};
}
static int fit_last_launch(const FitCall& c) { return c.valid ? c.n_epochs : c.n_epochs - 1; }

static int fit_closing_tail(const FitCall& c, int fin, int parity) {
  const Finishes w = launch_finishes(c, fit_last_launch(c) + 1);
  return fit_tail(c, fin, !c.valid, c.valid, w.adam_step, w.hist_index, w.valid_index, parity);
}

static int fit_pull(const FitCall& c, int parity) {
  const ndq_fused_fit* f = c.f;
  const ndq_fused_step& s0 = f->net[0];
  const int last = fit_last_launch(c);
  for (int e = 0; e <= last; ++e) {
    ndq::PullArgs pa{};
    if (e >= 1) {
      const Finishes w = launch_finishes(c, e);
      const int in = (e - 1) & 1, out = e & 1;
      pa.enabled = 1; pa.n_nets = f->n_nets; pa.nparts = s0.blocks;
      pa.lpart = c.LP[in]; pa.nlparts = s0.blocks; pa.lscale = s0.seed;
      pa.loss_hist = s0.loss_hist; pa.hist_index = w.hist_index; pa.loss_slot = s0.loss_slot;
      pa.vpart = w.with_valid ? c.VP[in] : nullptr; pa.nvparts = f->valid_blocks; pa.vscale = f->valid_scale;
      pa.valid_hist = f->valid_hist; pa.valid_index = w.valid_index; pa.best_on_valid = f->track_best == 2 ? 1 : 0;
      pa.best_loss = s0.best_loss; pa.parity = parity;
      const bool track = fit_tracks(f, true, w.with_valid);
      for (int k = 0; k < f->n_nets; ++k) {
        const ndq_fused_step& s = f->net[k];
        ndq::PullNet& n = pa.net[k];
        n.part = c.PART[in][k];
        n.p_in = c.P[in][k]; n.m_in = c.M[in][k]; n.v_in = c.V[in][k];
        n.p_out = c.P[out][k]; n.m_out = c.M[out][k]; n.v_out = c.V[out][k];
        n.grad = s.grad; n.best_flat = track ? s.best_flat : nullptr; n.len = s.n_params;
        n.adam = adam_consts(s.lr, s.beta1, s.beta2, s.eps, s.weight_decay, w.adam_step);
      }
      parity ^= 1;
    }
    const bool train_part = e < c.n_epochs, valid_part = c.valid && e >= 1;
    if (train_part && !c.train_coords[e]) return NDQ_EINVAL;
    int rc = f->launch(train_part ? c.train_coords[e] : nullptr, s0.ldc, train_part ? s0.n : 0, c.P[e & 1],
                       train_part ? c.PART[e & 1] : nullptr, c.LP[e & 1], s0.seed, valid_part ? f->valid_coords : nullptr,
                       f->valid_ldc, valid_part ? f->valid_n : 0, c.VP[e & 1], &pa, c.stream);
    if (rc) return rc;
  }
  return fit_closing_tail(c, last & 1, parity);
}

static int fit_loop(const FitCall& c, long long stride, int parity) {
  const ndq_fused_fit* f = c.f;
  const ndq_fused_step& s0 = f->net[0];
  const int last = fit_last_launch(c);
  int in = 0;
  for (int e0 = 0; e0 <= last; e0 += ndq::kLoopMaxLaunches, in ^= 1) {
    const int e1 = e0 + ndq::kLoopMaxLaunches <= last + 1 ? e0 + ndq::kLoopMaxLaunches : last + 1;
    const int out = in ^ 1;
    ndq::LoopArgs L{};
    L.e0 = e0; L.e1 = e1; L.n_epochs = c.n_epochs; L.has_valid = c.valid ? 1 : 0; L.track_best = f->track_best;
    L.hist_index = c.hist_index; L.valid_index = c.valid_index; L.parity = parity; L.coord_stride = stride;
    L.lp_in = c.LP[in]; L.vp_in = c.VP[in]; L.lp_out = c.LP[out]; L.vp_out = c.VP[out];
    L.lscale = s0.seed; L.vscale = f->valid_scale;
    L.loss_hist = s0.loss_hist; L.loss_slot = s0.loss_slot; L.valid_hist = f->valid_hist; L.best_loss = s0.best_loss;
    for (int k = 0; k < f->n_nets; ++k) {
      const ndq_fused_step& s = f->net[k];
      ndq::LoopNet& n = L.net[k];
      n.p_in = c.P[in][k]; n.m_in = c.M[in][k]; n.v_in = c.V[in][k]; n.part_in = c.PART[in][k];
      n.p_out = c.P[out][k]; n.m_out = c.M[out][k]; n.v_out = c.V[out][k]; n.part_out = c.PART[out][k];
      n.grad = s.grad; n.best_flat = s.best_flat;
      n.lr = s.lr; n.b1 = s.beta1; n.b2 = s.beta2; n.eps = s.eps; n.wd = s.weight_decay;
      for (int e = e0 > 1 ? e0 : 1; e < e1; ++e) {
        const ndq::AdamConsts a = adam_consts(s.lr, s.beta1, s.beta2, s.eps, s.weight_decay, launch_finishes(c, e).adam_step);
        n.bc1[e - e0] = a.bc1; n.bc2s[e - e0] = a.bc2s;
      }
// ... 160 lines not shown
```

neurodiffeq_amd/csrc/ndq_closure_host.h:

```cpp
#pragma once
#include <cstdlib>
#include <type_traits>

namespace {

template <class T> int fused_blocks(int n) {
  const int units = (n + T::POINTS - 1) / T::POINTS;
  int b = (units + T::SLOTS - 1) / T::SLOTS;
  return b > NDQ_MAX_BLOCKS ? NDQ_MAX_BLOCKS : (b < 1 ? 1 : b);
}

const ndq::real* g_theta = nullptr;
ndq::real* g_theta_partials = nullptr;

template <int K> void fill(ndq::FusedArgs& a, const ndq::real* const* params, ndq::real* const* partials) {
  a.params = params[0]; a.partials = partials ? partials[0] : nullptr;
}
template <int K> void fill(ndq::FusedMultiArgs& a, const ndq::real* const* params, ndq::real* const* partials) {
  for (int k = 0; k < K; ++k) { a.params[k] = params[k]; a.partials[k] = partials ? partials[k] : nullptr; }
}

template <class T>
int launch(const ndq::real* coords, int ldc, int n, const ndq::real* const* params, ndq::real* const* partials,
           ndq::real* loss_partials, ndq::real* funcs, ndq::real* resid, int ldj, ndq::real seed, int train, void* stream) {
  if (!coords || !params || !loss_partials || n <= 0 || ldc < n || (train && !partials)) return -2;
  if (T::Pw::NT > 0 && !g_theta) return -2;
  typename T::Args a{};
  a.coords = coords; a.loss_partials = loss_partials;
  fill<T::K>(a, params, partials);
  a.funcs = funcs; a.resid = resid; a.n = n; a.ldc = ldc; a.ldj = ldj; a.seed = seed;
  a.theta = g_theta; a.theta_partials = train ? g_theta_partials : nullptr;
  hipStream_t s = static_cast<hipStream_t>(stream);
  static bool attr = false;
  if (!attr) {
    hipError_t e = hipFuncSetAttribute(reinterpret_cast<const void*>(T::train),
                                       hipFuncAttributeMaxDynamicSharedMemorySize, (int)T::LDS_TRAIN);
    if (e != hipSuccess) return (int)e;
    e = hipFuncSetAttribute(reinterpret_cast<const void*>(T::eval),
                            hipFuncAttributeMaxDynamicSharedMemorySize, (int)T::LDS_EVAL);
    if (e != hipSuccess) return (int)e;
    attr = true;
  }
  if (train)
    hipLaunchKernelGGL(T::train, dim3(fused_blocks<T>(n)), dim3(T::THREADS), T::LDS_TRAIN, s, a);
  else
    hipLaunchKernelGGL(T::eval, dim3(fused_blocks<T>(n)), dim3(T::THREADS), T::LDS_EVAL, s, a);
  return (int)hipGetLastError();
}

template <class T>
int launch_tv(const ndq::real* coords, int ldc, int n, const ndq::real* const* params, ndq::real* const* partials,
              ndq::real* loss_partials, ndq::real seed, const ndq::real* vcoords, int vldc, int vn,
              ndq::real* vloss_partials, const void* pull, void* stream) {
  if (!params || n < 0 || vn < 0 || (n == 0 && vn == 0)) return -2;
  if (n > 0 && (!coords || !partials || !loss_partials || ldc < n)) return -2;
  if (vn > 0 && (!vcoords || !vloss_partials || vldc < vn)) return -2;
  typename T::Args t{}, v{};
  t.coords = coords; t.loss_partials = loss_partials; t.n = n; t.ldc = ldc; t.ldj = ldc; t.seed = seed;
  t.theta = g_theta; t.theta_partials = g_theta_partials;
  fill<T::K>(t, params, partials);
  v.coords = vcoords; v.loss_partials = vloss_partials; v.n = vn; v.ldc = vldc; v.ldj = vldc; v.seed = 0.f;
  v.theta = g_theta;
  fill<T::K>(v, params, nullptr);
  static const bool always_tv = getenv("NDQ_TV_ALWAYS") != nullptr;
  if (vn == 0 && !pull && !always_tv)
    return launch<T>(coords, ldc, n, params, partials, loss_partials, nullptr, nullptr, ldc, seed, 1, stream);
  const int tb = n > 0 ? fused_blocks<T>(n) : 0, vb = vn > 0 ? fused_blocks<T>(vn) : 0;
  static bool attr = false;
  if (!attr) {
    hipError_t e = hipFuncSetAttribute(reinterpret_cast<const void*>(T::tv),
                                       hipFuncAttributeMaxDynamicSharedMemorySize, (int)T::LDS_TRAIN);
    if (e != hipSuccess) return (int)e;
    attr = true;
  }
  ndq::PullArgs pa{};
  if (pull) {
    if (!ndq::pull_supported<typename T::Cfg>()) return -2;
    pa = *static_cast<const ndq::PullArgs*>(pull);
  }
  hipLaunchKernelGGL(T::tv, dim3(tb + vb), dim3(T::THREADS), tb > 0 ? T::LDS_TRAIN : T::LDS_EVAL,
                     static_cast<hipStream_t>(stream), t, v, tb, pa);
  return (int)hipGetLastError();
}

template <class T> constexpr bool has_loop() { return !std::is_same_v<std::remove_cv_t<decltype(T::loop)>, std::nullptr_t>; }

template <class T>
int launch_loop(const ndq::real* coords, int ldc, int n, ndq::real seed, const ndq::real* vcoords, int vldc, int vn,
                const void* loop, void* stream) {
  if constexpr (!has_loop<T>()) {
    return -2;
  } else {
    if (!loop || !ndq::pull_supported<typename T::Cfg>() || n < 0 || vn < 0 ||
        (n > 0 && (!coords || ldc < n || fused_blocks<T>(n) != 1)) ||
        (vn > 0 && (!vcoords || vldc < vn || fused_blocks<T>(vn) != 1)))
      return -2;
    typename T::Args t{}, v{};
    t.coords = coords; t.n = n; t.ldc = ldc; t.ldj = ldc; t.seed = seed; t.theta = g_theta;
    v.coords = vcoords; v.n = vn; v.ldc = vldc; v.ldj = vldc; v.seed = 0.f; v.theta = g_theta;
    static bool attr = false;
    if (!attr) {
      hipError_t e = hipFuncSetAttribute(reinterpret_cast<const void*>(T::loop),
                                         hipFuncAttributeMaxDynamicSharedMemorySize, (int)T::LDS_LOOP);
      if (e != hipSuccess) return (int)e;
      attr = true;
    }
    hipLaunchKernelGGL(T::loop, dim3(1), dim3(T::THREADS), T::LDS_LOOP, static_cast<hipStream_t>(stream), t, v,
                       *static_cast<const ndq::LoopArgs*>(loop));
    return (int)hipGetLastError();
  }
}
template <class T> int loop_ok() {
  return has_loop<T>() && ndq::pull_supported<typename T::Cfg>() && T::LDS_LOOP <= 160 * 1024 ? 1 : 0;
}

}

extern "C" int ndq_fused_blocks(int n) { return fused_blocks<Closure>(n); }
extern "C" int ndq_fused_num_params() { return Closure::Cfg::P; }
extern "C" int ndq_fused_num_theta() { return Closure::Pw::NT; }
extern "C" void ndq_fused_bind_theta(const ndq::real* theta, ndq::real* theta_partials) {
  g_theta = theta; g_theta_partials = theta_partials;
}
extern "C" int ndq_fused_num_nets() { return Closure::K; }
extern "C" int ndq_fused_threads() { return Closure::THREADS; }
extern "C" unsigned long ndq_fused_lds_bytes() { return (unsigned long)Closure::LDS_TRAIN; }

#ifdef NDQ_PHASE_TS
extern "C" int ndq_fused_phase_ts(unsigned long long* out) {
  return (int)hipMemcpyFromSymbol(out, HIP_SYMBOL(ndq::ndq_phase_ts), sizeof(unsigned long long) * 256 * 8);
}
extern "C" int ndq_fused_pull_ts(unsigned long long* out) {
  return (int)hipMemcpyFromSymbol(out, HIP_SYMBOL(ndq::ndq_pull_ts), sizeof(unsigned long long) * 8);
}
extern "C" int ndq_fused_tile_ts(unsigned long long* out) {
  return (int)hipMemcpyFromSymbol(out, HIP_SYMBOL(ndq::ndq_tile_ts), sizeof(unsigned long long) * 48);
}
#endif

extern "C" int ndq_fused_launch(const ndq::real* coords, int ldc, int n, const ndq::real* params, ndq::real* partials,
                                ndq::real* loss_partials, ndq::real* funcs, ndq::real* resid, int ldj, ndq::real seed,
                                int train, void* stream) {
  if (Closure::K != 1) return -2;
  const ndq::real* pp[1] = {params};
  ndq::real* qq[1] = {partials};
  return launch<Closure>(coords, ldc, n, pp, partials ? qq : nullptr, loss_partials, funcs, resid, ldj, seed, train, stream);
}

extern "C" int ndq_fused_launch_multi(const ndq::real* coords, int ldc, int n, const ndq::real* const* params,
                                      ndq::real* const* partials, ndq::real* loss_partials, ndq::real* funcs,
                                      ndq::real* resid, int ldj, ndq::real seed, int train, void* stream) {
  return launch<Closure>(coords, ldc, n, params, partials, loss_partials, funcs, resid, ldj, seed, train, stream);
}

extern "C" int ndq_fused_launch_tv(const ndq::real* coords, int ldc, int n, const ndq::real* const* params,
                                   ndq::real* const* partials, ndq::real* loss_partials, ndq::real seed,
                                   const ndq::real* vcoords, int vldc, int vn, ndq::real* vloss_partials, const void* pull,
                                   void* stream) {
  return launch_tv<Closure>(coords, ldc, n, params, partials, loss_partials, seed, vcoords, vldc, vn, vloss_partials, pull, stream);
}
extern "C" int ndq_fused_pull_ok() { return ndq::pull_supported<Closure::Cfg>() ? 1 : 0; }
extern "C" int ndq_fused_launch_loop(const ndq::real* coords, int ldc, int n, ndq::real seed, const ndq::real* vcoords,
                                     int vldc, int vn, const void* loop, void* stream) {
  return launch_loop<Closure>(coords, ldc, n, seed, vcoords, vldc, vn, loop, stream);
}
extern "C" int ndq_fused_loop_ok() { return loop_ok<Closure>(); }
```

neurodiffeq_amd/csrc/ndq_mlp.h:

```cpp
#pragma once
#include <hip/hip_runtime.h>
#include <utility>
#include <type_traits>
#include "ndq_tail.h"

namespace ndq {

#ifndef NDQ_F64
#define NDQ_F64 0
#endif
#if NDQ_F64
typedef double real;
#else
typedef float real;
#endif
typedef real real4 __attribute__((ext_vector_type(4)));

#if NDQ_F64
__device__ __forceinline__ real rfma(real a, real b, real c) { return fma(a, b, c); }
#else
__device__ __forceinline__ real rfma(real a, real b, real c) { return fmaf(a, b, c); }
#endif
__device__ __forceinline__ real4 mfma16x16x4(real a, real b, real4 c) {
#if NDQ_F64
// ... 230 lines not shown
#endif
#ifndef NDQ_FWD_NPROD
#define NDQ_FWD_NPROD 6
#endif
#ifndef NDQ_HBAR_NPROD
#define NDQ_HBAR_NPROD 6
#endif
#ifndef NDQ_WG_NPROD
#define NDQ_WG_NPROD 6
#endif
#define NDQ_PRODUCTS_6(T) T(a1, 1) T(a2, 0) T(a0, 2) T(a1, 0) T(a0, 1) T(a0, 0)
#define NDQ_PRODUCTS_5(T) T(a1, 1) T(a2, 0) T(a1, 0) T(a0, 1) T(a0, 0)
#define NDQ_PRODUCTS_4(T) T(a2, 0) T(a1, 0) T(a0, 1) T(a0, 0)
#define NDQ_PRODUCTS_3(T) T(a1, 0) T(a0, 1) T(a0, 0)
#define NDQ_CAT_(a, b) a##b
#define NDQ_CAT(a, b) NDQ_CAT_(a, b)
#define NDQ_PRODUCTS_FWD(T) NDQ_CAT(NDQ_PRODUCTS_, NDQ_FWD_NPROD)(T)
#define NDQ_PRODUCTS_BWD(T) NDQ_CAT(NDQ_PRODUCTS_, NDQ_HBAR_NPROD)(T)
#if NDQ_FWD_NPROD < 3 || NDQ_FWD_NPROD > 6 || NDQ_HBAR_NPROD < 3 || NDQ_HBAR_NPROD > 6
#error "NDQ_FWD_NPROD / NDQ_HBAR_NPROD must be 3, 4, 5 or 6"
#endif
#if NDQ_WG_NPROD == 6
#define NDQ_WPRODUCTS(W) W(1, 1) W(2, 0) W(0, 2) W(1, 0) W(0, 1) W(0, 0)
#elif NDQ_WG_NPROD == 4
#define NDQ_WPRODUCTS(W) W(1, 1) W(1, 0) W(0, 1) W(0, 0)
#elif NDQ_WG_NPROD == 3
#define NDQ_WPRODUCTS(W) W(1, 0) W(0, 1) W(0, 0)
#else
#error "NDQ_WG_NPROD must be 3, 4 or 6"
#endif
#define NDQ_HTR_PLANES ((NDQ_WG_NPROD == 6) ? 3 : 2)
#define NDQ_H_PLANES ((NDQ_FWD_NPROD == 6 || NDQ_WG_NPROD == 6) ? 3 : 2)
#define NDQ_Z_PLANES ((NDQ_HBAR_NPROD == 6 || NDQ_WG_NPROD == 6) ? 3 : 2)
#ifndef NDQ_WIDE_LOWREG
#define NDQ_WIDE_LOWREG 1
#endif
#ifndef NDQ_PIN_WEIGHT_READS
#define NDQ_PIN_WEIGHT_READS 1
#endif
#ifndef NDQ_WIDE_SG
#define NDQ_WIDE_SG 2
#endif
#ifndef NDQ_KEEP_H
#define NDQ_KEEP_H 1
#endif
#ifndef NDQ_FWD_THREADS
#define NDQ_FWD_THREADS 256
#endif
#ifndef NDQ_WG_SCHED_BARRIER
#define NDQ_WG_SCHED_BARRIER 1
#endif
#ifndef NDQ_WIDE_LAUNDER
#define NDQ_WIDE_LAUNDER 1
#endif
#ifndef NDQ_WG_BF16
#define NDQ_WG_BF16 0
#endif
#ifndef NDQ_WG_TR
#define NDQ_WG_TR 0
#endif
#ifndef NDQ_MULTI_G2
#define NDQ_MULTI_G2 2
#endif
#ifndef NDQ_WG_TR_K
#define NDQ_WG_TR_K 1
#endif
#ifndef NDQ_FWD_BF16X1
#define NDQ_FWD_BF16X1 0
#endif
#ifndef NDQ_QUAD_SWAP
#define NDQ_QUAD_SWAP 1
#endif
#ifndef NDQ_SPLIT_PAIRS
#define NDQ_SPLIT_PAIRS 0
#endif
#ifndef NDQ_WG32
#define NDQ_WG32 1
#endif
#ifndef NDQ_ABL
#define NDQ_ABL 0
#endif
#ifndef NDQ_STAGE_INFLIGHT
#define NDQ_STAGE_INFLIGHT 1
#endif
#ifndef NDQ_GROUP_PREFETCH
#define NDQ_GROUP_PREFETCH 1
#endif
#ifndef NDQ_STAGGER
#define NDQ_STAGGER 0
#endif

__device__ __forceinline__ real tanh_fast(real z) {
#if NDQ_F64
  return tanh(z);
#else
  const real e = __builtin_amdgcn_exp2f(z * 2.88539008177792681472f);
  return rfma(-2.f, __builtin_amdgcn_rcpf(e + 1.f), 1.f);
#endif
}

template <int ACT> struct Act;
template <> struct Act<ACT_TANH> {
  static __device__ __forceinline__ void fwd(real z, real& t, real& c, real = 1.f) {
#if NDQ_FAST_TANH || NDQ_F64
    t = tanh_fast(z);
#else
    t = tanhf(z);
#endif
    c = 0.f;
  }
  static __device__ __forceinline__ real s1(real t, real, real = 1.f) { return rfma(-t, t, 1.f); }
  static __device__ __forceinline__ real s2(real t, real, real s1v) { return -2.f * t * s1v; }
  static __device__ __forceinline__ real s3(real, real, real s1v) { return s1v * rfma(-6.f, s1v, 4.f); }
  static __device__ __forceinline__ real s4(real t, real, real s1v) { return t * s1v * rfma(24.f, s1v, -8.f); }
  static __device__ __forceinline__ real s5(real, real, real s1v) { return s1v * rfma(s1v, rfma(120.f, s1v, -120.f), 16.f); }
};
template <> struct Act<ACT_SIN> {
  static __device__ __forceinline__ void fwd(real z, real& t, real& c, real = 1.f) {
#if NDQ_F64
    sincos(z, &t, &c);
#else
    sincosf(z, &t, &c);
#endif
  }
  static __device__ __forceinline__ real s1(real, real c, real = 1.f) { return c; }
  static __device__ __forceinline__ real s2(real t, real, real) { return -t; }
  static __device__ __forceinline__ real s3(real, real c, real) { return -c; }
  static __device__ __forceinline__ real s4(real t, real, real) { return t; }
  static __device__ __forceinline__ real s5(real, real c, real) { return c; }
};

__device__ __forceinline__ real sigmoid_fast(real z) {
#if NDQ_F64
  return 1.0 / (1.0 + exp(-z));
#else
  return __builtin_amdgcn_rcpf(1.f + __builtin_amdgcn_exp2f(-1.4426950408889634f * z));
#endif
}
template <> struct Act<ACT_SIGMOID> {
  static __device__ __forceinline__ void fwd(real z, real& t, real& c, real = 1.f) { t = sigmoid_fast(z); c = 0.f; }
  static __device__ __forceinline__ real s1(real t, real, real = 1.f) { return t * (1.f - t); }
  static __device__ __forceinline__ real s2(real t, real, real s1v) { return s1v * rfma(-2.f, t, 1.f); }
  static __device__ __forceinline__ real s3(real, real, real s1v) { return s1v * rfma(-6.f, s1v, 1.f); }
  static __device__ __forceinline__ real s4(real t, real, real s1v) {
    return s1v * rfma(-2.f, t, 1.f) * rfma(-12.f, s1v, 1.f);
  }
  static __device__ __forceinline__ real s5(real, real, real s1v) { return s1v * rfma(s1v, rfma(120.f, s1v, -30.f), 1.f); }
};
template <> struct Act<ACT_SWISH> {
  static __device__ __forceinline__ void fwd(real z, real& t, real& c, real = 1.f) { c = sigmoid_fast(z); t = z * c; }
  static __device__ __forceinline__ real s1(real t, real c, real = 1.f) { return rfma(t, 1.f - c, c); }
  static __device__ __forceinline__ real s2(real t, real c, real) {
    return (1.f - c) * rfma(t, rfma(-2.f, c, 1.f), 2.f * c);
  }
  static __device__ __forceinline__ real s3(real t, real c, real) {
    return (1.f - c) * rfma(t, rfma(6.f * c, c - 1.f, 1.f), 3.f * c * rfma(-2.f, c, 1.f));
  }
};

template <> struct Act<ACT_APTX> {
  static __device__ __forceinline__ void fwd(real z, real& t, real& c, real al = 1.f) { c = z; t = 0.5f * z * (al + tanh_fast(z)); }
  static __device__ __forceinline__ real s1(real, real z, real al = 1.f) {
    const real T = tanh_fast(z);
    return 0.5f * rfma(z, rfma(-T, T, 1.f), al + T);
  }
  static __device__ __forceinline__ real s2(real, real z, real) {
// ... 111 lines not shown
  static constexpr int offS = offbout + NOUT;
  static constexpr int ACTP = ACTP_;
  static constexpr int AK = (ACT_ == ACT_SWISH) ? 1 : (ACT_ == ACT_APTX) ? 3 : 0;
  static_assert(ACTP_ == 0 || AK > 0, "trainable activation parameters: Swish / APTx");
  static constexpr bool ALPHA = (ACTP_ != 0) && (ACT_ == ACT_APTX);
  static constexpr int offA = offS + SKIP * NOUT * D;
  static constexpr int P = offA + (ACTP_ == 1 ? AK * L : 0);
  static constexpr int ldsW1T = 0, ldsb1 = NIN * H;
  static constexpr int ldsLayer0 = NIN * H + H;
  static constexpr bool BF16 = (NDQ_BF16X3 != 0) && (NB_ % 2 == 0) && (NDQ_F64 == 0);
  static constexpr int NC = NB_ / 2;
  static constexpr int WEL = BF16 ? (H * H * 3) / 2 : H * H;
  static constexpr bool BF16O = BF16 && (NOUT_ > 1) && (NBO % 2 == 0);
  static constexpr int NCO = NBO / 2;
  static constexpr int WOEL = BF16O ? (HO * H * 3) / 2 : HO * H;
  static constexpr bool KEEP_H = (NB_ == 2) && (NDQ_KEEP_H != 0) && (SS::NS <= 6) && (BWD_THREADS == 256);
  static constexpr bool LAUNDER = ((NB_ == 2) && (BWD_THREADS != 256)) || (NB_ >= 4 && NDQ_WIDE_LAUNDER);
  static constexpr bool WIDE = (NB_ >= 4) && (NDQ_WIDE_LOWREG != 0);
  static constexpr bool GROUP_HBAR = WIDE || (BWD_THREADS != 256 && SS::NS > 2);
  static constexpr int SG = GROUP_HBAR ? NDQ_WIDE_SG : SS::NS;
  static constexpr bool ACC_LDS = WIDE && (NOUT_ == 1);
  static constexpr int biasFloats = ACC_LDS ? H * (D_ + L_ + 1) : 0;
  static constexpr int biasB1 = 0, biasW1 = H, biasBl = H * (1 + D_), biasWout = H * (D_ + L_);
  static constexpr int layerStride(bool bwd) { return (bwd ? 2 : 1) * WEL + H; }
  static constexpr int ldsWf(int l, bool bwd) { return ldsLayer0 + (l - 2) * layerStride(bwd); }
  static constexpr int ldsWt(int l) { return ldsWf(l, true) + WEL; }
  static constexpr int ldsb(int l, bool bwd) { return ldsWf(l, bwd) + (bwd ? 2 : 1) * WEL; }
  static constexpr int ldsWout(bool bwd) { return ldsLayer0 + (L - 1) * layerStride(bwd); }
  static constexpr int ldsWoutT() { return ldsWout(true) + WOEL; }
  static constexpr int ldsbout(bool bwd) { return ldsWout(bwd) + (NOUT == 1 ? H : (bwd ? 2 : 1) * WOEL); }
  static constexpr int ldsSkip(bool bwd) { return ldsbout(bwd) + (NOUT == 1 ? 1 : HO); }
  static constexpr int ldsAlpha(bool bwd) { return ldsSkip(bwd) + SKIP * D * (NOUT == 1 ? 1 : HO); }
  static constexpr int ldsWeightsEnd(bool bwd) { return (ldsAlpha(bwd) + (ALPHA ? L : 0) + 3) & ~3; }
  static constexpr bool WG_BF16 = BF16 && (NB_ <= 2) && (NDQ_WG_BF16 != 0);
  static constexpr bool WG32 = BF16 && (NB_ == 4) && (NDQ_WG32 != 0);
  static constexpr int WG_SB = (NB_ <= 2 && SS::NS >= 2 && (BWD_THREADS == 256 || WG_BF16)) ? 2 : 1;
  static constexpr int stageFloatsPlain = WG_SB * 2 * 16 * HP;
  static constexpr int trPlane = 256;
  static constexpr int trHimg = (L_ - 1) * SS::NS * 3 * trPlane;
  static constexpr int trStage = trHimg + 2 * 3 * trPlane;
  static constexpr int trWaves = NDQ_WG_TR_K == 1 ? BWD_THREADS / 64 : (NDQ_WG_TR_K == 2 ? NDQ_MULTI_G2 : 1);
  static constexpr bool WG_TR = BF16 && (NB_ == 2) && (L_ >= 2) && (NOUT_ == 1) && (NDQ_WG_TR != 0) && !WG_BF16 &&
                                (NDQ_WG_TR_K * (ldsWeightsEnd(true) + trWaves * trStage) +
                                 (NDQ_WG_TR_K > 1 ? 2 * trWaves * NDQ_WG_TR_K * SS::NS * 16 : 0) + 64 <= 40 * 1024);
  static constexpr int trPlane64 = 512;
  static constexpr int trStage64 = 2 * 3 * trPlane64;
  static constexpr bool WG_TR64 = WG32 && (NOUT_ == 1) && (NDQ_WG_TR != 0) && (NDQ_WG_TR_K == 1) &&
                                  (ldsWeightsEnd(true) + (BWD_THREADS / 64) * (trStage64 + biasFloats) + 64 <= 40 * 1024);
  static constexpr int stageFloatsPerWave = WG_TR ? trStage : WG_TR64 ? trStage64 : stageFloatsPlain;
};

struct MlpArgs {
  const real* coords;
  const real* params;
  const real* gbar;
  real* jets;
  real* partials;
  int n;
  int ldc;
  int ldj;
};

template <class C>
__device__ __forceinline__ real act_pre(const real* __restrict__ prm, int l) {
  if constexpr (C::ACTP == 0) return 1.f;
  else return prm[C::offA + (l - 1) * C::AK + (C::AK == 3 ? 1 : 0)];
}
template <class C>
__device__ __forceinline__ real act_post(const real* __restrict__ prm, int l) {
  if constexpr (C::ACTP == 0) return 1.f;
  else {
    if (l == 0) return 1.f;
    const real beta = act_pre<C>(prm, l);
    if constexpr (C::AK == 3) return 2.f * prm[C::offA + (l - 1) * 3 + 2] / beta;
    else return 1.f / beta;
  }
}
template <class C>
__device__ __forceinline__ real actp_mul(real v, real f) {
  if constexpr (C::ACTP != 0) return v * f;
  else return v;
}

template <class C, bool BWD>
__device__ __forceinline__ void stage_weights(real* lds, const real* __restrict__ prm, int tid = -1, int nt = 0) {
  constexpr int H = C::H, D = C::D, NB = C::NB;
  constexpr int HL = C::hr(C::L);
  if (tid < 0) { tid = threadIdx.x; nt = blockDim.x; }
  const real f1 = act_pre<C>(prm, 1), fo = act_post<C>(prm, C::L);
  auto unit = [&](int j, int hw, int idx, real f) {
    if constexpr (C::RAGGED) return j < hw ? actp_mul<C>(prm[idx], f) : (real)0.f;
    else return actp_mul<C>(prm[idx], f);
  };
  auto real_unit = [](int j, int hw) { return !C::RAGGED || j < hw; };
#if NDQ_STAGE_INFLIGHT
  if constexpr (C::ACTP == 0 && !C::RAGGED && C::MONO == 0 && C::SKIP == 0 && C::BF16 && (C::NOUT == 1 || C::BF16O)) {
    constexpr int KP = 8, P = C::P, LS = H * H + H;
    auto place_wout = [&](int j, int k, real w) {
      __bf16* wf = reinterpret_cast<__bf16*>(lds + C::ldsWout(BWD));
      __bf16* wt = reinterpret_cast<__bf16*>(lds + C::ldsWoutT());
      const __bf16 w0 = (__bf16)w; const real r1 = w - (real)w0;
      const __bf16 w1 = (__bf16)r1; const __bf16 w2 = (__bf16)(r1 - (real)w1);
      {
        const int blk = (j >> 4) * C::NC + (k >> 5);
        const int base = ((blk * 3) * 64 + (j & 15) + 16 * ((k & 15) >> 2)) * 8 + 4 * ((k & 31) >> 4) + (k & 3);
        wf[base] = w0; wf[base + 512] = w1; wf[base + 1024] = w2;
      }
      if (BWD) {
        const int blk = (k >> 4) * C::NCO + (j >> 5);
        const int base = ((blk * 3) * 64 + (k & 15) + 16 * ((j & 15) >> 2)) * 8 + 4 * ((j & 31) >> 4) + (j & 3);
        wt[base] = w0; wt[base + 512] = w1; wt[base + 1024] = w2;
      }
    };
    if constexpr (C::NOUT > 1) {
      for (int i = C::NOUT * H + tid; i < C::HO * H; i += nt) place_wout(i / H, i % H, (real)0.f);
      for (int i = C::NOUT + tid; i < C::HO; i += nt) lds[C::ldsbout(BWD) + i] = 0.f;
    }
    auto place = [&](int e, real w) {
      if (e < C::offb1) {
        const int j = e / C::NIN, a = e - j * C::NIN;
        lds[C::ldsW1T + a * H + j] = w;
      } else if (e < C::offW(2)) {
        lds[C::ldsb1 + (e - C::offb1)] = w;
      } else if (e < C::offWout) {
        const int l = 2 + (e - C::offW(2)) / LS, r = (e - C::offW(2)) % LS;
        if (r >= H * H) { lds[C::ldsb(l, BWD) + (r - H * H)] = w; return; }
        const int j = r / H, k = r - j * H;
        __bf16* wf = reinterpret_cast<__bf16*>(lds + C::ldsWf(l, BWD));
        __bf16* wt = reinterpret_cast<__bf16*>(lds + C::ldsWt(l));
        const __bf16 w0 = (__bf16)w; const real r1 = w - (real)w0;
        const __bf16 w1 = (__bf16)r1; const __bf16 w2 = (__bf16)(r1 - (real)w1);
        {
          const int blk = (j >> 4) * C::NC + (k >> 5);
          const int base = ((blk * 3) * 64 + (j & 15) + 16 * ((k & 15) >> 2)) * 8 + 4 * ((k & 31) >> 4) + (k & 3);
          wf[base] = w0; wf[base + 512] = w1; wf[base + 1024] = w2;
        }
        if (BWD) {
          const int blk = (k >> 4) * C::NC + (j >> 5);
          const int base = ((blk * 3) * 64 + (k & 15) + 16 * ((j & 15) >> 2)) * 8 + 4 * ((j & 31) >> 4) + (j & 3);
          wt[base] = w0; wt[base + 512] = w1; wt[base + 1024] = w2;
        }
      } else if (e < C::offbout) {
        if constexpr (C::NOUT == 1) lds[C::ldsWout(BWD) + (e - C::offWout)] = w;
        else place_wout((e - C::offWout) / H, (e - C::offWout) % H, w);
      } else {
        lds[C::ldsbout(BWD) + (e - C::offbout)] = w;
      }
    };
    for (int base = 0; base < P; base += KP * nt) {
      real v[KP];
#pragma unroll
      for (int k = 0; k < KP; ++k) {
        const int e = base + tid + k * nt;
        v[k] = prm[e < P ? e : P - 1];
      }
      asm volatile("" : "+v"(v[0]), "+v"(v[1]), "+v"(v[2]), "+v"(v[3]), "+v"(v[4]), "+v"(v[5]), "+v"(v[6]), "+v"(v[7]));
#pragma unroll
      for (int k = 0; k < KP; ++k) {
        const int e = base + tid + k * nt;
        if (e < P) place(e, v[k]);
      }
    }
    return;
  }
#endif
  for (int i = tid; i < C::NIN * H; i += nt) {
    const int a = i / H, j = i - a * H;
    lds[C::ldsW1T + i] = unit(j, C::hr(1), C::offW1 + j * C::NIN + a, f1);
  }
  for (int i = tid; i < H; i += nt) lds[C::ldsb1 + i] = unit(i, C::hr(1), C::offb1 + i, f1);
  if constexpr (C::ALPHA) {
    if (tid < C::L) lds[C::ldsAlpha(BWD) + tid] = prm[C::offA + 3 * tid];
  }
  if constexpr (C::SKIP != 0 && C::NOUT > 1) {
    for (int i = tid; i < D * C::HO; i += nt) {
      const int a = i / C::HO, u = i - a * C::HO;
      lds[C::ldsSkip(BWD) + i] = u < C::NOUT ? prm[C::offS + u * D + a] : 0.f;
    }
  }
  if constexpr (C::NOUT == 1) {
    for (int i = tid; i < H; i += nt) lds[C::ldsWout(BWD) + i] = unit(i, HL, C::offWout + i, fo);
    if (tid == 0) lds[C::ldsbout(BWD)] = prm[C::offbout];
    if constexpr (C::SKIP != 0) {
      if (tid < D) lds[C::ldsSkip(BWD) + tid] = prm[C::offS + tid];
    }
  } else if constexpr (C::BF16O) {
    const real* Wo = prm + C::offWout;
    __bf16* wf = reinterpret_cast<__bf16*>(lds + C::ldsWout(BWD));
    __bf16* wt = reinterpret_cast<__bf16*>(lds + C::ldsWoutT());
    for (int i = tid; i < C::HO * H; i += nt) {
      const int j = i / H, k = i - j * H;
      real w;
      if constexpr (C::RAGGED) w = (j < C::NOUT && k < HL) ? actp_mul<C>(Wo[j * HL + k], fo) : 0.f;
      else w = j < C::NOUT ? actp_mul<C>(Wo[i], fo) : 0.f;
      const __bf16 w0 = (__bf16)w; const real r1 = w - (real)w0;
      const __bf16 w1 = (__bf16)r1; const __bf16 w2 = (__bf16)(r1 - (real)w1);
      {
        const int blk = (j >> 4) * C::NC + (k >> 5);
        const int base = ((blk * 3) * 64 + (j & 15) + 16 * ((k & 15) >> 2)) * 8 + 4 * ((k & 31) >> 4) + (k & 3);
        wf[base] = w0; wf[base + 512] = w1; wf[base + 1024] = w2;
      }
      if (BWD) {
        const int blk = (k >> 4) * C::NCO + (j >> 5);
        const int base = ((blk * 3) * 64 + (k & 15) + 16 * ((j & 15) >> 2)) * 8 + 4 * ((j & 31) >> 4) + (j & 3);
        wt[base] = w0; wt[base + 512] = w1; wt[base + 1024] = w2;
      }
    }
    for (int i = tid; i < C::HO; i += nt) lds[C::ldsbout(BWD) + i] = i < C::NOUT ? prm[C::offbout + i] : 0.f;
  } else {
    constexpr int NBO = C::NBO;
    const real* Wo = prm + C::offWout;
    for (int i = tid; i < C::HO * H; i += nt) {
      const int lane = i & 63, t = (i >> 6) & 3, blk = i >> 8;
      {
        const int ob = blk / NB, kb = blk - ob * NB;
        const int o = 16 * ob + mrow(lane & 15);
        const int k = 16 * kb + 4 * (lane >> 4) + t;
        lds[C::ldsWout(BWD) + i] = (o < C::NOUT && real_unit(k, HL)) ? actp_mul<C>(Wo[o * HL + k], fo) : 0.f;
      }
      if (BWD) {
        const int kb = blk / NBO, ob = blk - kb * NBO;
        const int o = 16 * ob + 4 * (lane >> 4) + t;
        const int k = 16 * kb + mrow(lane & 15);
        lds[C::ldsWoutT() + i] = (o < C::NOUT && real_unit(k, HL)) ? actp_mul<C>(Wo[o * HL + k], fo) : 0.f;
      }
    }
    for (int i = tid; i < C::HO; i += nt) lds[C::ldsbout(BWD) + i] = i < C::NOUT ? prm[C::offbout + i] : 0.f;
  }
  if constexpr (C::BF16) {
#pragma unroll
    for (int l = 2; l <= C::L; ++l) {
// ... 1782 lines not shown
}

template <class C>
__global__ __launch_bounds__(C::BWD_THREADS) void mlp_jet_bwd_kernel(MlpArgs a) {
  extern __shared__ __attribute__((aligned(16))) real lds[];
  const int lane = threadIdx.x & 63, wave = threadIdx.x >> 6, p = lane & 15, q = lane >> 4;
  constexpr int WAVES = C::BWD_THREADS / 64;
  const int ntiles = (a.n + 15) >> 4;
  real xn[C::D], gn[C::NOUT == 1 ? C::NS : 1];
  {
    const int n0 = (blockIdx.x * WAVES + wave) * 16 + p;
    const int nn0 = n0 < a.n ? n0 : a.n - 1;
#pragma unroll
    for (int d = 0; d < C::D; ++d) xn[d] = a.coords[(size_t)d * a.ldc + nn0];
    if constexpr (C::NOUT == 1) {
#pragma unroll
      for (int s = 0; s < C::NS; ++s) gn[s] = a.gbar[(size_t)s * a.ldj + nn0];
    }
  }
  stage_weights<C, true>(lds, a.params);
  __syncthreads();
  real* stage = lds + C::ldsWeightsEnd(true) + wave * C::stageFloatsPerWave;
  GradAcc<C> acc;
  acc_init<C>(acc, lds, WAVES, wave, lane);
  for (int tile = blockIdx.x * WAVES + wave; tile < ntiles; tile += gridDim.x * WAVES) {
    const int n = tile * 16 + p;
    const bool valid = n < a.n;
    const int nn = valid ? n : a.n - 1;
    real x[C::D], gcur[C::NOUT == 1 ? C::NS : 1];
#pragma unroll
    for (int d = 0; d < C::D; ++d) x[d] = xn[d];
    if constexpr (C::NOUT == 1) {
#pragma unroll
      for (int s = 0; s < C::NS; ++s) gcur[s] = gn[s];
    }
    {
      const int n1 = n + gridDim.x * WAVES * 16;
      const int nn1 = n1 < a.n ? n1 : a.n - 1;
#pragma unroll
      for (int d = 0; d < C::D; ++d) xn[d] = a.coords[(size_t)d * a.ldc + nn1];
      if constexpr (C::NOUT == 1) {
#pragma unroll
        for (int s = 0; s < C::NS; ++s) gn[s] = a.gbar[(size_t)s * a.ldj + nn1];
      }
    }
    const real* ldsw = lds + opaque_zero<C>();
    LayerState<C> st[C::L];
    real4 h[C::NS][C::NB];
    KeptPlanes<C> kp;
    tile_forward<C, true>(ldsw, lane, q, x, st, h, kp, stage);
    if constexpr (C::NOUT == 1) {
      real gout[C::NS];
#pragma unroll
      for (int s = 0; s < C::NS; ++s) gout[s] = valid ? gcur[s] : 0.f;
      tile_backward<C>(ldsw, stage, lane, p, q, x, gout, st, acc, kp);
    } else {
      real4 go[C::NS][C::NBO];
#pragma unroll
      for (int s = 0; s < C::NS; ++s)
#pragma unroll
        for (int ob = 0; ob < C::NBO; ++ob)
#pragma unroll
          for (int r = 0; r < 4; ++r) {
            const int u = 16 * ob + 4 * q + r;
            go[s][ob][r] = (valid && u < C::NOUT) ? a.gbar[((size_t)s * C::NOUT + u) * a.ldj + nn] : 0.f;
          }
      tile_backward_multi<C>(ldsw, stage, lane, p, q, x, go, st, acc, kp);
    }
  }
  block_reduce_store<C, WAVES>(lds, acc, wave, lane, p, q, a.partials + (size_t)blockIdx.x * C::P, a.params);
}

struct FusedArgs {
  const real* coords;
  const real* params;
  real* partials;
  real* loss_partials;
  real* funcs;
  real* resid;
  int n, ldc, ldj;
  real seed;
  const real* theta;
  real* theta_partials;
};

template <int NT>
__device__ __forceinline__ void theta_block_sum(real (&t)[NT > 0 ? NT : 1], real* scratch, int waves, real* out) {
  if constexpr (NT > 0) {
    const int lane = threadIdx.x & 63, wave = threadIdx.x >> 6;
#pragma unroll
    for (int j = 0; j < NT; ++j) t[j] = point_sum(quad_sum(t[j]));
    __syncthreads();
    if (lane == 0) {
#pragma unroll
      for (int j = 0; j < NT; ++j) scratch[wave * NT + j] = t[j];
    }
    __syncthreads();
    if ((int)threadIdx.x < NT && out) {
      real v = 0.f;
      for (int w = 0; w < waves; ++w) v += scratch[w * NT + threadIdx.x];
      out[threadIdx.x] = v;
    }
  }
}

template <class C, class = void> struct no_pull_marker : std::false_type {};
template <class C> struct no_pull_marker<C, std::void_t<decltype(C::NO_PULL)>> : std::true_type {};
template <class C> constexpr bool pull_supported() { return NDQ_F64 == 0 && C::ACTP == 0 && !no_pull_marker<C>::value; }
template <class C> constexpr int pull_floats() { return ((C::P + 3) & ~3) + 32; }

template <class C, class PW, bool TRAIN>
__device__ __forceinline__ void fused_closure_body(const FusedArgs& a, real* lds, const int blk, const int nblk,
                                                   const PullArgs& pull, bool writer) {
  static_assert(C::NOUT == 1, "the single-launch closure kernel needs a single-output network");
  NDQ_TS(0);
#ifdef NDQ_PHASE_TS
  if (threadIdx.x == 0 && blockIdx.x == 0) ndq_tile_iter = 0;
#endif
  const int lane = threadIdx.x & 63, wave = threadIdx.x >> 6, p = lane & 15, q = lane >> 4;
  constexpr int WAVES = C::BWD_THREADS / 64;
  const int ntiles = (a.n + 15) >> 4;
  real xn[C::D];
  {
    const int n0 = (blk * WAVES + wave) * 16 + p;
    const int nn0 = n0 < a.n ? n0 : a.n - 1;
#pragma unroll
    for (int d = 0; d < C::D; ++d) xn[d] = a.coords[(size_t)d * a.ldc + nn0];
  }
  const real* prm = a.params;
#if !NDQ_F64
  if constexpr (pull_supported<C>()) {
    if (pull.enabled) {
      float* pnew = lds + C::ldsWeightsEnd(TRAIN);
      NDQ_PT(0);
#ifdef NDQ_PHASE_TS
      if (threadIdx.x == 0 && blockIdx.x == 0) {
        ndq_pull_ts[4] = ndq_phase_ts[4 + 3];
        ndq_pull_ts[5] = ndq_phase_ts[8 + 4 + 3];
      }
#endif
      pull_prologue<C::BWD_THREADS, C::P, 1>(pull, pnew, 0, pnew + ((C::P + 3) & ~3), writer);
      NDQ_PT(2);
      __syncthreads();
      prm = pnew;
    }
  }
#endif
  stage_weights<C, TRAIN>(lds, prm);
  __syncthreads();
  NDQ_PT(3);
  NDQ_TS(1);
  real* stage = lds + C::ldsWeightsEnd(true) + wave * C::stageFloatsPerWave;
  GradAcc<C> acc;
  if constexpr (TRAIN) acc_init<C>(acc, lds, WAVES, wave, lane);
  real lsum = 0.f;
  constexpr int NXE = PW::ND + PW::NT;
  real xe[NXE > 0 ? NXE : 1], tsum[PW::NT > 0 ? PW::NT : 1];
#pragma unroll
  for (int j = 0; j < PW::NT; ++j) { xe[PW::ND + j] = a.theta[j]; tsum[j] = 0.f; }
#if NDQ_STAGGER > 0
  if (WAVES > 4 && wave >= WAVES / 2) __builtin_amdgcn_s_sleep(NDQ_STAGGER);
#endif
  for (int tile = blk * WAVES + wave; tile < ntiles; tile += nblk * WAVES) {
    const int n = tile * 16 + p;
    const bool valid = n < a.n;
    real x[C::D];
#pragma unroll
    for (int d = 0; d < C::D; ++d) x[d] = xn[d];
    {
      const int n1 = n + nblk * WAVES * 16;
      const int nn1 = n1 < a.n ? n1 : a.n - 1;
#pragma unroll
      for (int d = 0; d < C::D; ++d) xn[d] = a.coords[(size_t)d * a.ldc + nn1];
    }
    const real* ldsw = lds + opaque_zero<C>();
    LayerState<C> st[C::L];
    real4 h[C::NS][C::NB];
    KeptPlanes<C> kp;
    NDQ_TT(0);
    tile_forward<C, TRAIN>(ldsw, lane, q, x, st, h, kp, stage);
    NDQ_TT(1);
    real jets[C::NS], gout[C::NS], r[PW::NR], f[PW::NF > 0 ? PW::NF : 1], gth[PW::NT > 0 ? PW::NT : 1];
    tile_output<C, TRAIN>(ldsw, q, x, h, jets);
    NDQ_TT(2);
    if constexpr (PW::ND > 0) {
      const int nn = valid ? n : a.n - 1;
#pragma unroll
      for (int j = 0; j < PW::ND; ++j) xe[j] = a.coords[(size_t)(C::D + j) * a.ldc + nn];
    }
    PW::apply(x, xe, jets, a.seed, TRAIN ? 1 : 0, r, f, gout, gth);
    NDQ_TT(3);
    if (valid && q == 0) {
      lsum += PW::loss(r);
      if constexpr (TRAIN) {
#pragma unroll
        for (int j = 0; j < PW::NT; ++j) tsum[j] += gth[j];
      }
      if (a.resid) {
#pragma unroll
        for (int e = 0; e < PW::NEQ; ++e) a.resid[(size_t)e * a.ldj + n] = r[e];
      }
      if (a.funcs) {
#pragma unroll
        for (int m = 0; m < PW::NF; ++m) a.funcs[(size_t)m * a.ldj + n] = f[m];
      }
    }
    if constexpr (TRAIN) {
#pragma unroll
      for (int s = 0; s < C::NS; ++s) gout[s] = valid ? gout[s] : 0.f;
      tile_backward<C>(ldsw, stage, lane, p, q, x, gout, st, acc, kp);
    }
    NDQ_TT(12);
#ifdef NDQ_PHASE_TS
    if (threadIdx.x == 0 && blockIdx.x == 0) ndq_tile_iter = 1;
#endif
  }
#ifdef NDQ_PHASE_TS
  __syncthreads();
  NDQ_TS(2);
#endif
  if constexpr (TRAIN) block_reduce_store<C, WAVES>(lds, acc, wave, lane, p, q, a.partials + (size_t)blk * C::P, a.params);
  lsum = point_sum(quad_sum(lsum));
  __syncthreads();
  real* wl = lds + C::ldsWeightsEnd(TRAIN);
  if (lane == 0) wl[wave] = lsum;
  __syncthreads();
  if (threadIdx.x == 0) {
    real v = 0.f;
    for (int w = 0; w < WAVES; ++w) v += wl[w];
    a.loss_partials[blk] = v;
  }
  if constexpr (TRAIN) theta_block_sum<PW::NT>(tsum, wl + 16, WAVES, a.theta_partials ? a.theta_partials + (size_t)blk * PW::NT : nullptr);
  NDQ_TS(3);
}

template <class C, class PW, bool TRAIN>
__global__ __launch_bounds__(C::BWD_THREADS) void fused_closure_kernel(FusedArgs a) {
  extern __shared__ __attribute__((aligned(16))) real lds[];
  const PullArgs none{};
  fused_closure_body<C, PW, TRAIN>(a, lds, blockIdx.x, gridDim.x, none, false);
}

template <class C, class PW>
__global__ __launch_bounds__(C::BWD_THREADS) void fused_closure_tv_kernel(FusedArgs t, FusedArgs v, int train_blocks, PullArgs pull) {
  extern __shared__ __attribute__((aligned(16))) real lds[];
  const bool writer = blockIdx.x == 0;
  if ((int)blockIdx.x < train_blocks) fused_closure_body<C, PW, true>(t, lds, blockIdx.x, train_blocks, pull, writer);
  else fused_closure_body<C, PW, false>(v, lds, (int)blockIdx.x - train_blocks, (int)gridDim.x - train_blocks, pull, writer);
}

template <class C> constexpr size_t fused_lds_bytes(bool train);
template <class C> constexpr int loop_state_offset() {
  const size_t a = fused_lds_bytes<C>(true), b = fused_lds_bytes<C>(false);
  return (int)((((a > b ? a : b) + 15) & ~(size_t)15) / sizeof(real));
}
template <class C> constexpr int loop_state_floats(int nets) { return nets * 4 * ((C::P + 3) & ~3) + 64; }
template <class C> constexpr size_t fused_loop_lds_bytes() { return sizeof(real) * (loop_state_offset<C>() + loop_state_floats<C>(1)); }

template <int K>
__device__ __forceinline__ void loop_state_load(const LoopArgs& L, float* state, int pp, int len, float* misc) {
#pragma unroll
  for (int k = 0; k < K; ++k) {
    float* s = state + (size_t)k * 4 * pp;
    for (int i = threadIdx.x; i < len; i += blockDim.x) {
      s[i] = L.net[k].p_in[i];
      s[pp + i] = L.net[k].m_in[i];
      s[2 * pp + i] = L.net[k].v_in[i];
      s[3 * pp + i] = L.e0 >= 1 ? L.net[k].part_in[i] : 0.f;
    }
  }
  if (threadIdx.x == 0) {
    misc[0] = L.e0 >= 1 ? L.lp_in[0] : 0.f;
    misc[1] = (L.e0 >= 2 && L.has_valid) ? L.vp_in[0] : 0.f;
    misc[2] = L.best_loss[0];
    misc[3] = L.best_loss[1];
  }
}
template <int K>
__device__ __forceinline__ void loop_state_store(const LoopArgs& L, const float* state, int pp, int len, const float* misc) {
#pragma unroll
  for (int k = 0; k < K; ++k) {
    const float* s = state + (size_t)k * 4 * pp;
    for (int i = threadIdx.x; i < len; i += blockDim.x) {
      L.net[k].p_out[i] = s[i];
      L.net[k].m_out[i] = s[pp + i];
      L.net[k].v_out[i] = s[2 * pp + i];
      L.net[k].part_out[i] = s[3 * pp + i];
    }
  }
  if (threadIdx.x == 0) {
    L.lp_out[0] = misc[0];
    if (L.has_valid) L.vp_out[0] = misc[1];
    L.best_loss[0] = misc[2];
    L.best_loss[1] = misc[3];
  }
}

#if !NDQ_F64
template <class C, class PW>
__global__ __launch_bounds__(C::BWD_THREADS) void fused_closure_loop_kernel(FusedArgs t, FusedArgs v, LoopArgs L) {
  extern __shared__ __attribute__((aligned(16))) real lds[];
  if constexpr (!pull_supported<C>()) return;
  constexpr int PP = (C::P + 3) & ~3;
  float* state = lds + loop_state_offset<C>();
  float* misc = state + 4 * PP;
  const PullArgs none{};
  loop_state_load<1>(L, state, PP, C::P, misc);
  __syncthreads();
  for (int e = L.e0; e < L.e1; ++e) {
    if (e >= 1) {
      PullArgs pa{};
      loop_pull_args<1>(L, e, state, PP, C::P, misc, pa);
      pull_prologue<C::BWD_THREADS, C::P, 1>(pa, state, 0, misc + 8, true);
      __syncthreads();
    }
    if (L.has_valid && e >= 1) {
      FusedArgs a = v;
      a.params = state; a.loss_partials = misc + 1;
      fused_closure_body<C, PW, false>(a, lds, 0, 1, none, false);
      __syncthreads();
    }
    if (e < L.n_epochs) {
      FusedArgs a = t;
// ... 478 lines not shown
```

neurodiffeq_amd/engine.py:

```python
import ctypes
import os

import torch

from . import _lib, codegen, generators
from .networks import FlatParams, describe
from .symbolic import Graph, Sym, TraceUnsupported, trace_scope

_c_vp = ctypes.c_void_p


def _ptr(t):
    return _c_vp(t.data_ptr())


_raw_stream = getattr(torch._C, "_cuda_getCurrentRawStream", None) or \
    (lambda idx: torch.cuda.current_stream(idx).cuda_stream)


def _round_up(n, m):
    return (n + m - 1) // m * m


class _Lib64:
# ... 780 lines not shown
            if with_train:
                ok = ok and torch.equal(lp, want_loss) and all(torch.equal(a, w) for a, w in zip(parts, want_parts))
            if with_valid:
                ok = ok and torch.equal(vp, ev)
        return bool(ok)

    SELF_CHECK_TOL = 2e-5

    def reject_fused(self):
        self.fusedk, self.fusedk_wide, self._fast = None, False, None
        self._bufs.clear()
        self._resident_cache.clear()

    def verify_on(self, batch, n_global=None, lo=0, hi=None):
        b, n = self.upload(batch, lo, hi)
        self.set_batch_size(n if n_global is None else n_global)
        self.refresh_theta()
        ok = self.verify_fused(b, n, n_global)
        if batch[0].device.type != "cuda":
            self._static_seen.pop(self.static_key(batch) + (lo, batch[0].numel() if hi is None else hi), None)
        return ok

    def fused_closure(self, b, n, stream, train, n_global, slot, accumulate, want_funcs=False, want_resid=False):
        for fp in self.flat:
            fp.sync()
        seed = 1.0 / (float(n_global) * self.loss_norm)
        params_pp = (_c_vp * len(self.flat))(*[fp.flat.data_ptr() for fp in self.flat])
        self._bind_theta(b, b["fusedk"].lib, True)
        rc = b["fusedk"].lib.ndq_fused_launch_multi(self._coord_ptr(b, 0), b["ld"], n, params_pp,
                                                    b["fused_partials_pp"] if train else None,
                                                    _ptr(b["fused_loss_partials"]),
                                                    _ptr(b["funcs"]) if want_funcs else None,
                                                    _ptr(b["resid"]) if want_resid else None, b["ld"], seed,
                                                    1 if train else 0, stream)
        _lib.check(rc, "ndq_fused_launch_multi")
        if train:
            for fp, part in zip(self.flat, b["fused_partials_all"]):
                rc = self.L.ndq_reduce_partials(_ptr(part), b["fused_blocks"], fp.numel, _ptr(fp.grad),
                                                1 if accumulate else 0, 1.0, stream)
                _lib.check(rc, "ndq_reduce_partials")
            self.reduce_theta(b, b["fused_blocks"], stream, accumulate)
        rc = self.L.ndq_reduce_partials(_ptr(b["fused_loss_partials"]), b["fused_blocks"], 1,
                                        _c_vp(self.loss_buf.data_ptr() + self.esize * slot), 0, seed, stream)
        _lib.check(rc, "ndq_reduce_partials(loss)")

    HIST = 8192

    def fast_ready(self, dist=None):
        return self.fusedk is not None and (len(self.nets) == 1 or dist is None) and not self.f64 and not self.n_theta

    def launches_per_step(self):
        if self.fusedk is not None and self.f64:
            return 4
        if self.fusedk is not None:
            return 2
        total = 1 + 1 + len(self.flat)
        for k in range(self.n_sites):
            d = self.descs[k]
            if d.hidden > 64 and d.layers >= 2:
                wide_head = 1 if d.hidden > 128 else 0
                total += (1 + (d.layers - 1) + wide_head) + (wide_head + 2 * (d.layers - 1) + 1) + 1
            else:
                total += 1 + 2
        return total

    def fast_state(self):
        if getattr(self, "_fast", None) is None:
            dev, f32 = self.device, self.dt
            self._fast = dict(loss_hist=torch.zeros(self.HIST, dtype=f32, device=dev),
                              valid_hist=torch.zeros(self.HIST, dtype=f32, device=dev),
                              best_loss=torch.full((2,), float("inf"), dtype=f32, device=dev),
                              best_flat=[torch.zeros_like(fp.grad) for fp in self.flat], parity=0, pending=0,
                              pending_valid=0, structs={})
        return self._fast

    def _fill_step(self, st, k, n, ld, blocks, partials, loss_partials):
        fs, fp = self.fast_state(), self.flat[k]
        st.n, st.ldc, st.ldj, st.blocks, st.n_params = n, ld, ld, blocks, fp.numel
        if partials is not None:
            st.partials, st.loss_partials = partials.data_ptr(), loss_partials.data_ptr()
        st.grad, st.loss_slot = fp.grad.data_ptr(), fp.grad_loss.data_ptr() + 4 * fp.numel
        st.loss_hist, st.best_loss = fs["loss_hist"].data_ptr(), fs["best_loss"].data_ptr()

    @staticmethod
    def _set_adam(st, m, v, group):
        st.adam_m, st.adam_v = m.data_ptr(), v.data_ptr()
        (st.beta1, st.beta2), st.lr, st.eps, st.weight_decay = group["betas"], group["lr"], group["eps"], group["weight_decay"]

    @staticmethod
    def _tail_args(fp, adam_slot):
        if adam_slot is None:
            return _ptr(fp.flat), None, None, None, fp.numel, 0.0, 0.0, 0.0, 0.0, 0.0, 1
        m, v, group, step = adam_slot
        return (_ptr(fp.flat), _ptr(fp.grad), _ptr(m), _ptr(v), fp.numel, group["lr"], *group["betas"], group["eps"],
                group["weight_decay"], step)

    def epoch_tail(self, kind, n_batches, track_best, adam_slots=None):
        fs = self.fast_state()
        stream = self._stream()
        train = kind == "train"
        hist = fs["loss_hist"] if train else fs["valid_hist"]
        idx = fs["pending"] if train else fs["pending_valid"]
        parity = fs["parity"]
        for k, fp in enumerate(self.flat):
            fp.sync()
            args = self._tail_args(fp, adam_slots[k] if train else None)
            rc = self.L.ndq_epoch_tail(*args, _ptr(self.loss_buf), n_batches, _ptr(hist), idx, _ptr(fs["best_loss"]),
                                       parity, _ptr(fs["best_flat"][k]) if track_best else None, 1 if k == 0 else 0,
                                       stream)
            _lib.check(rc, "ndq_epoch_tail")
        if train:
            fs["pending"] += 1
        else:
            fs["pending_valid"] += 1
        fs["parity"] ^= 1

    def fast_train_epoch_multi(self, batch, adam_slots, track_best):
        fs = self.fast_state()
        b, n = self.upload(batch)
        K = len(self.flat)
        key = (n, b["ld"], id(b), "multi")
        arr = fs["structs"].get(key)
        if arr is None:
            arr = (_lib.FusedStep * K)()
            for k in range(K):
                self._fill_step(arr[k], k, n, b["ld"], b["fused_blocks"], b["fused_partials_all"][k], b["fused_loss_partials"])
            fs["structs"][key] = arr
        step = None
        for k, fp in enumerate(self.flat):
            fp.sync()
            m, v, group, step_k = adam_slots[k]
            step = step_k if step is None else step
            st = arr[k]
            st.params = fp.flat.data_ptr()
            st.seed = 1.0 / (float(n) * self.loss_norm)
            st.best_flat = fs["best_flat"][k].data_ptr() if track_best else None
            self._set_adam(st, m, v, group)
        rc = self.L.ndq_fused_multi_step_run(arr, K, _c_vp(b["fused_launch_multi"]), self._coord_ptr(b, 0), step,
                                             fs["pending"], fs["parity"], self._stream())
        _lib.check(rc, "ndq_fused_multi_step_run")
        fs["pending"] += 1
        fs["parity"] ^= 1

    def fast_train_epoch(self, batch, optimizer, adam_slot, track_best, n_global=None, dist=None):
        fs = self.fast_state()
        b, n = self.upload(batch)
        fp = self.flat[0]
        fp.sync()
        m, v, group, step = adam_slot
        key = (n, b["ld"], id(b))
        st = fs["structs"].get(key)
        if st is None:
            st = _lib.FusedStep()
            st.launch = b["fused_launch"]
            self._fill_step(st, 0, n, b["ld"], b["fused_blocks"], b["fused_partials"], b["fused_loss_partials"])
            fs["structs"][key] = st
        n_global = n if n_global is None else n_global
        st.params = fp.flat.data_ptr()
        st.seed = 1.0 / (float(n_global) * self.loss_norm)
        st.best_flat = fs["best_flat"][0].data_ptr() if track_best else None
        self._set_adam(st, m, v, group)
        stream = self._stream()
        coords = self._coord_ptr(b, 0)
        hist_index, parity = fs["pending"], fs["parity"]
        src = generators.device_source(batch) if dist is None else None
        if src is not None and src.prefetch and b["coords_rows"] is not None:
            st.next_sampler = ctypes.addressof(src.desc)
            st.next_seed, st.next_draw, st.next_stream = src.seed, src.draw, src.stream_id
            nxt = src.block_of(src.draw)
            st.next_coords, st.next_ldc = nxt.data_ptr(), nxt.shape[1]
        else:
            src, st.next_sampler = None, None
        direct = dist.direct(self.device, fp.numel + 1) if dist is not None else None
        if dist is None or direct is not None:
            st.allreduce, st.comm = direct if direct is not None else (None, None)
            rc = self.L.ndq_fused_step_run(ctypes.byref(st), coords, step, hist_index, parity, stream)
            _lib.check(rc, "ndq_fused_step_run")
            if src is not None:
                src.prefetched = src.draw
        else:
            st.adam_m = st.adam_v = None
            st.allreduce = st.comm = None
            rc = self.L.ndq_fused_step_run(ctypes.byref(st), coords, step, hist_index, parity, stream)
            _lib.check(rc, "ndq_fused_step_run")
            dist.all_reduce_flat(fp.grad_loss)
            rc = self.L.ndq_epoch_tail(*self._tail_args(fp, adam_slot), _c_vp(st.loss_slot), 1, _ptr(fs["loss_hist"]),
                                       hist_index, _ptr(fs["best_loss"]), parity,
                                       _ptr(fs["best_flat"][0]) if track_best else None, 1, stream)
            _lib.check(rc, "ndq_epoch_tail")
        fs["pending"] += 1
        fs["parity"] ^= 1

    FIT_RUN = os.environ.get("NDQ_FIT_RUN", "1") != "0"
    FIT_PULL = os.environ.get("NDQ_FIT_PULL", "1") != "0"
    FIT_LOOP = os.environ.get("NDQ_FIT_LOOP", "1") != "0"

    def fit_ready(self):
        return self.FIT_RUN and self.fusedk is not None and not self.f64 and not self.n_theta

    def resident_ptr(self, batch):
        if batch[0].device.type != "cuda" or len(batch) != self.n_coords:
            return None
        ld = self._resident_ld(batch)
        return (batch[0].data_ptr(), ld) if ld else None

    def stage_batches(self, host_block, n, reserve=0):
        K = host_block.shape[0]
        ld = _round_up(n, 64)
        st = self.__dict__.setdefault("_stage", dict(pinned=[None, None], events=[None, None], next=0, dev=[None, None]))
        i = st["next"]
        st["next"] ^= 1
        need = K * self.n_coords * ld
        if st["pinned"][i] is None or st["pinned"][i].numel() < need:
            if st["events"][i] is not None:
                st["events"][i].synchronize()
            size = max(need, reserve * self.n_coords * ld)
            for j in (0, 1):
                if st["pinned"][j] is None or st["pinned"][j].numel() < size:
                    if st["events"][j] is not None:
                        st["events"][j].synchronize()
                    st["pinned"][j] = torch.zeros(size, dtype=torch.float32, device="cpu", pin_memory=True)
                    st["dev"][j] = torch.zeros(size, dtype=torch.float32, device=self.device)
        elif st["events"][i] is not None:
            st["events"][i].synchronize()
        pinned = st["pinned"][i][:need].view(K, self.n_coords, ld)
        import numpy as np
        np.copyto(pinned.numpy()[:, :, :n], host_block.detach().numpy(), casting="same_kind")
        dev = st["dev"][i][:need].view(K, self.n_coords, ld)
        dev.copy_(pinned, non_blocking=True)
        ev = st["events"][i] or torch.cuda.Event()
        ev.record()
        st["events"][i] = ev
        return dev, ld

    def fit_run(self, train_ptrs, n, ld, adam_slots, valid=None, track_best=0, n_global=None):
        fs = self.fast_state()
        K = len(train_ptrs)
        if K:
            self._fit_last_n = n
        fk = self.fused_variant(n if K else (getattr(self, "_fit_last_n", None) or valid[1]))
        key = (id(fk), n if K else 0, ld if K else 0, (valid[1], valid[2]) if valid else None)
        cache = fs.setdefault("fit", {})
        ent = cache.get(key)
        if ent is None:
            if len(cache) >= 8:
                cache.pop(next(iter(cache)))
            dev, f32 = self.device, torch.float32
            ff = _lib.FusedFit()
            ff.launch = ctypes.cast(fk.lib.ndq_fused_launch_tv, ctypes.c_void_p).value
            ff.n_nets = len(self.flat)
            keep = []
            blocks = fk.blocks(n) if K else 0
            lparts = torch.zeros(max(blocks, 1), dtype=f32, device=dev)
            keep.append(lparts)
            for k, fp in enumerate(self.flat):
                part = torch.empty(blocks, fp.numel, dtype=f32, device=dev) if K else None
                keep.append(part)
                self._fill_step(ff.net[k], k, *((n, ld, blocks) if K else (0, 0, 0)), part, lparts)
                ff.net[k].best_flat = fs["best_flat"][k].data_ptr()
            if valid is not None:
                vparts = torch.zeros(fk.blocks(valid[1]), dtype=f32, device=dev)
                keep.append(vparts)
                ff.valid_n, ff.valid_ldc, ff.valid_blocks = valid[1], valid[2], vparts.numel()
                ff.valid_scale = 1.0 / (float(valid[1]) * self.loss_norm)
                ff.valid_loss_partials, ff.valid_hist = vparts.data_ptr(), fs["valid_hist"].data_ptr()
            ff.pull_ok = 0
            if K and self.FIT_PULL and 0 < blocks * len(self.flat) <= 16 and fk.lib.ndq_fused_pull_ok():
                ff.pull_ok = 1
                for k, fp in enumerate(self.flat):
                    alt = [torch.zeros(fp.numel, dtype=f32, device=dev) for _ in range(3)]
                    apart = torch.empty(blocks, fp.numel, dtype=f32, device=dev)
                    keep.extend(alt + [apart])
                    ff.alt_params[k], ff.alt_m[k], ff.alt_v[k] = (t.data_ptr() for t in alt)
                    ff.alt_partials[k] = apart.data_ptr()
                alp = torch.zeros(max(blocks, 1), dtype=f32, device=dev)
                keep.append(alp)
                ff.alt_loss_partials = alp.data_ptr()
                if valid is not None:
                    avp = torch.zeros(ff.valid_blocks, dtype=f32, device=dev)
                    keep.append(avp)
                    ff.alt_valid_loss_partials = avp.data_ptr()
                if self.FIT_LOOP and blocks == 1 and (valid is None or ff.valid_blocks == 1) and len(self.flat) <= 2 \
                        and fk.lib.ndq_fused_loop_ok():
                    ff.launch_loop = ctypes.cast(fk.lib.ndq_fused_launch_loop, ctypes.c_void_p).value
                    ff.loop_ok = 1
            ent = cache[key] = (ff, keep, fk, {}, (_c_vp * 1)(), ctypes.byref(ff))
        ff = ent[0]
        step0 = 1
        last = ent[3]
        for k, fp in enumerate(self.flat):
            fp.sync()
            if K:
                m, v, group, step0 = adam_slots[k]
                now = (fp.flat.data_ptr(), n if n_global is None else n_global, m.data_ptr(), v.data_ptr(), group["lr"],
                       group["betas"], group["eps"], group["weight_decay"])
            else:
                now = (fp.flat.data_ptr(),)
            if last.get(k) != now:
                last[k] = now
                st = ff.net[k]
                st.params = now[0]
                if K:
                    st.seed = 1.0 / (float(now[1]) * self.loss_norm)
                    self._set_adam(st, m, v, group)
        vc = valid[0] if valid is not None else None
        if last.get("v") != (vc, track_best):
            last["v"] = (vc, track_best)
            ff.valid_coords = vc
            ff.track_best = track_best
        if K == 1:
            coords = ent[4]
            coords[0] = train_ptrs[0]
        else:
            coords = (_c_vp * max(K, 1))(*train_ptrs) if K else None
        rc = self.L.ndq_fused_fit_run(ent[5], K, coords, step0, fs["pending"], fs["pending_valid"], fs["parity"],
                                      self._stream())
        _lib.check(rc, "ndq_fused_fit_run")
        tails = K + (1 if valid is not None else 0)
        fs["pending"] += K
        if valid is not None:
            fs["pending_valid"] += max(K, 1)
        fs["parity"] ^= tails & 1

    def fast_flush(self):
        fs = getattr(self, "_fast", None)
        if fs is None or (fs["pending"] == 0 and fs["pending_valid"] == 0):
            return [], [], None
        k, kv = fs["pending"], fs["pending_valid"]
        vals = torch.cat([fs["loss_hist"][:k], fs["valid_hist"][:kv],
                          fs["best_loss"][fs["parity"]:fs["parity"] + 1]]).tolist()
        fs["pending"] = fs["pending_valid"] = 0
        return vals[:k], vals[k:k + kv], vals[k + kv]

    def step(self, batch, train, slot=0, accumulate=False, n_global=None, lo=0, hi=None, want_funcs=False,
             want_resid=False):
        b, n = self.upload(batch, lo, hi)
        n_global = n if n_global is None else n_global
        stream = self._stream()
        self.set_batch_size(n_global)
        self.refresh_theta()
        if train and not accumulate and not self.verify_fused(b, n, n_global):
            b, n = self.upload(batch, lo, hi)
# ... 11 lines not shown
```

Baseline: 3.052 billion collocation-points/s.

## Keep a pre-laid-out LDS weight image updated by the Adam tail

The Adam tail kernel now writes each updated parameter straight into a persistent global buffer. That buffer already has the fused kernel's shared-memory weight layout, including the bf16 split transposed tiles, and the tail also records a witness copy of the parameter. At startup, each closure block copies this image into LDS with vectorised loads and checks it against the live parameters through the witness. It only falls back to the full per-element stage_weights scatter if any block sees a mismatch. This targets the per-block cost of splitting and scattering the weights, and adds extra global reads, an OR-reduced barrier, and more scattered writes in the tail.

```diff
diff --git a/__graft_entry__.py b/__graft_entry__.py
--- a/__graft_entry__.py
+++ b/__graft_entry__.py
@@ -140,6 +140,24 @@
                 print("built", so, f"({name}: 8-wave build of the closure kernel)", flush=True)
     os.environ.pop("NDQ_FUSE_GROUP", None)
     os.environ.pop("NDQ_NO_LAP", None)
+    old_flags = os.environ.get("NDQ_JIT_FLAGS")
+    os.environ["NDQ_JIT_FLAGS"] = ((old_flags + " ") if old_flags else "") + "-DNDQ_WEIGHT_IMAGE=0"
+    try:
+        for name, nets, conds, pde, nc, cfv in systems[:4]:
+            assert name in ("c1", "c2", "c3", "c4")
+            if name == "c1":
+                continue
+            program, descs = trace_system(nets, conds, pde, nc, compute_func_val=cfv)
+            built.add(codegen.build(program))
+            built.add(codegen.build_fused(program, descs[0]))
+            if name == "c2":
+                built.add(codegen.build_fused(program, descs[0], threads=512))
+            print("built", name, "(closure kernels with in-kernel weight staging only)", flush=True)
+    finally:
+        if old_flags is None:
+            os.environ.pop("NDQ_JIT_FLAGS", None)
+        else:
+            os.environ["NDQ_JIT_FLAGS"] = old_flags
     f64_systems = []
     for name, size in (("c1", 8), ("c2", 8), ("c3", 8)):
         torch.manual_seed(0)
diff --git a/include/ndq.h b/include/ndq.h
--- a/include/ndq.h
+++ b/include/ndq.h
@@ -150,6 +150,11 @@
                                    float* loss_partials, float* funcs, float* resid, int ldj, float seed, int train,
                                    void* stream);
 
+typedef int (*ndq_fused_launch_image_fn)(const float* coords, int ldc, int n, const float* const* params,
+                                         float* const* partials, float* loss_partials, float seed,
+                                         const float* valid_coords, int valid_ldc, int valid_n, float* valid_loss_partials,
+                                         const float* image, const float* witness, int image_floats, void* stream);
+
 typedef int (*ndq_allreduce_fn)(const void* sendbuf, void* recvbuf, size_t count, int dtype, int op, void* comm,
                                 void* stream);
 
@@ -175,6 +180,11 @@
   unsigned next_stream;
   float* next_coords;
   int next_ldc;
+  ndq_fused_launch_image_fn launch_image;
+  float* image;
+  float* witness;
+  const int* image_table;
+  int image_floats;
 } ndq_fused_step;
 int ndq_fused_step_run(const ndq_fused_step* s, const float* coords, int adam_step, int hist_index, int parity,
                        void* stream);
diff --git a/neurodiffeq_amd/_lib.py b/neurodiffeq_amd/_lib.py
--- a/neurodiffeq_amd/_lib.py
+++ b/neurodiffeq_amd/_lib.py
@@ -81,7 +81,9 @@
                 ("loss_hist", ctypes.c_void_p), ("best_loss", ctypes.c_void_p), ("best_flat", ctypes.c_void_p),
                 ("allreduce", ctypes.c_void_p), ("comm", ctypes.c_void_p),
                 ("next_sampler", ctypes.c_void_p), ("next_seed", ctypes.c_ulonglong), ("next_draw", ctypes.c_ulonglong),
-                ("next_stream", ctypes.c_uint), ("next_coords", ctypes.c_void_p), ("next_ldc", ctypes.c_int)]
+                ("next_stream", ctypes.c_uint), ("next_coords", ctypes.c_void_p), ("next_ldc", ctypes.c_int),
+                ("launch_image", ctypes.c_void_p), ("image", ctypes.c_void_p), ("witness", ctypes.c_void_p),
+                ("image_table", ctypes.c_void_p), ("image_floats", ctypes.c_int)]
 
 
 class FusedFit(ctypes.Structure):
diff --git a/neurodiffeq_amd/codegen.py b/neurodiffeq_amd/codegen.py
--- a/neurodiffeq_amd/codegen.py
+++ b/neurodiffeq_amd/codegen.py
@@ -140,7 +140,7 @@
 }
 
 
-def _closure_host(K, threads, points, slots, kern, kern_tv, lds, kern_loop=None, lds_loop=None):
+def _closure_host(K, threads, points, slots, kern, kern_tv, lds, kern_loop=None, lds_loop=None, image=False):
     return f"""struct Closure {{
   using Cfg = CFG;
   using Pw = PW;
@@ -151,6 +151,7 @@
   static constexpr auto tv = &{kern_tv};
   static constexpr auto loop = {'&' + kern_loop if kern_loop else 'nullptr'};
   static constexpr size_t LDS_TRAIN = {lds('true')}, LDS_EVAL = {lds('false')}, LDS_LOOP = {lds_loop or 0};
+  static constexpr bool IMAGE = {'true' if image else 'false'};
 }};
 }}  // namespace
 #include "ndq_closure_host.h"
@@ -453,7 +454,7 @@
             kern_loop, lds_loop = f"ndq::fused_multi_closure_loop_kernel<CFG, {K}, PW>", f"(ndq::fused_multi_loop_lds_bytes<CFG, {K}>())"
         else:
             kern_loop = lds_loop = None
-        host = _closure_host(K, threads, 16, tiles_per_block, kern, kern_tv, lds, kern_loop, lds_loop)
+        host = _closure_host(K, threads, 16, tiles_per_block, kern, kern_tv, lds, kern_loop, lds_loop, image=(K == 1))
         wg_tr = f"#ifndef NDQ_WG_TR\n#define NDQ_WG_TR 1\n#endif\n#define NDQ_WG_TR_K {K}\n" + CLOSURE_PRODUCTS
         return f"""// GENERATED by neurodiffeq_amd/codegen.py -- single-launch closure kernel (forward streams + pointwise stage +
 // reverse pass) of one PDE system with {K} network(s), gfx950.
@@ -752,6 +753,13 @@
         self.lib.ndq_fused_launch_tv.restype = ci
         self.lib.ndq_fused_launch_tv.argtypes = [vp, ci, ci, vp, vp, vp, cf, vp, ci, ci, vp, vp, vp]
         self.lib.ndq_fused_pull_ok.restype = ci
+        self.lib.ndq_weight_image_floats.restype = ci
+        self.lib.ndq_weight_image_table.restype = ci
+        self.lib.ndq_weight_image_table.argtypes = [vp]
+        self.lib.ndq_weight_image_init.restype = ci
+        self.lib.ndq_weight_image_init.argtypes = [vp, vp, vp, vp]
+        self.lib.ndq_weight_image_launch.restype = ci
+        self.lib.ndq_weight_image_launch.argtypes = [vp, ci, ci, vp, vp, vp, cf, vp, ci, ci, vp, vp, vp, ci, vp]
         self.lib.ndq_fused_launch_loop.restype = ci
         self.lib.ndq_fused_launch_loop.argtypes = [vp, ci, ci, cf, vp, ci, ci, vp, vp]
         self.lib.ndq_fused_loop_ok.restype = ci
diff --git a/neurodiffeq_amd/csrc/ndq_api.hip b/neurodiffeq_amd/csrc/ndq_api.hip
--- a/neurodiffeq_amd/csrc/ndq_api.hip
+++ b/neurodiffeq_amd/csrc/ndq_api.hip
@@ -183,7 +183,11 @@
   int tail_blocks;
   ndq::SampleArgs smp;
   ValidArgs v;
+  float* image; float* witness; const int2* table; int image_floats;
 };
+#ifndef NDQ_WEIGHT_IMAGE
+#define NDQ_WEIGHT_IMAGE 1
+#endif
 #ifndef NDQ_TAIL_COLS
 #define NDQ_TAIL_COLS 64
 #endif
@@ -212,6 +216,9 @@
     if (has_train || a.t.p_in) { m0 = m_in[i]; v0 = v_in[i]; }
   }
   const float best = a.t.best_loss[a.t.parity];
+  const bool img = NDQ_WEIGHT_IMAGE != 0 && a.image != nullptr && has_train;
+  int2 dst = make_int2(-1, -1);
+  if (img && upd) dst = a.table[i];
   float lp = lp0, vp = vp0;
   for (int r = tid + TT; r < a.r.nlparts; r += TT) lp += a.r.lpart[r];
   if (has_valid)
@@ -247,6 +254,14 @@
       a.t.m[i] = mi;
       a.t.v[i] = vi;
       a.t.p[i] = pn;
+      if (img) {
+        const ndq::ImageDest d{dst.x, dst.y};
+        const int top = d.x < 0 ? ~d.x : (d.x > d.y ? d.x : d.y) / 2 + 512;
+        if (top < a.image_floats) {
+          ndq::image_put(a.image, d, pn);
+          a.witness[i] = pn;
+        }
+      }
     } else if (a.t.p_in) {
       a.t.p[i] = pi; a.t.m[i] = m0; a.t.v[i] = v0;
     }
@@ -454,8 +469,11 @@
 static ReduceTailArgs reduce_tail_args(const ndq_fused_step& s, const ndq_fused_step& s0, const float* part, const float* lpart,
                                        int nparts, int adam_step, int hist_index, int parity, int write_scalars,
                                        float* best_flat, const ValidArgs& v = ValidArgs{}, const float* p_in = nullptr,
-                                       const float* m_in = nullptr, const float* v_in = nullptr) {
+                                       const float* m_in = nullptr, const float* v_in = nullptr, bool image = false) {
   ReduceTailArgs a{};
+  if (image && s.image && s.witness && s.image_table && s.image_floats > 0) {
+    a.image = s.image; a.witness = s.witness; a.table = reinterpret_cast<const int2*>(s.image_table); a.image_floats = s.image_floats;
+  }
   a.r = Reduce2Args{part, nparts, s.n_params, s.grad, 0, lpart, nparts, s.loss_slot, s0.seed};
   a.t.p = s.params; a.t.g = s.grad; a.t.m = s.adam_m; a.t.v = s.adam_v; a.t.len = s.n_params;
   a.t.adam = adam_consts(s.lr, s.beta1, s.beta2, s.eps, s.weight_decay, adam_step);
@@ -467,13 +485,25 @@
   return a;
 }
 
+static bool step_image(const ndq_fused_step& s) {
+  return NDQ_WEIGHT_IMAGE != 0 && s.launch_image && s.image && s.witness && s.image_table && s.image_floats > 0;
+}
+
 extern "C" {
 
 int ndq_fused_step_run(const ndq_fused_step* s, const float* coords, int adam_step, int hist_index, int parity,
                        void* stream) {
   if (!s || !s->launch || !coords) return NDQ_EINVAL;
-  int rc = s->launch(coords, s->ldc, s->n, s->params, s->partials, s->loss_partials, nullptr, nullptr, s->ldj, s->seed,
-                     1, stream);
+  const bool image = step_image(*s) && s->adam_m && !s->allreduce;
+  int rc;
+  if (image) {
+    const float* pp[1] = {s->params};
+    float* qq[1] = {s->partials};
+    rc = s->launch_image(coords, s->ldc, s->n, pp, qq, s->loss_partials, s->seed, nullptr, 0, 0, nullptr, s->image, s->witness,
+                         s->image_floats, stream);
+  } else {
+    rc = s->launch(coords, s->ldc, s->n, s->params, s->partials, s->loss_partials, nullptr, nullptr, s->ldj, s->seed, 1, stream);
+  }
   if (rc) return rc;
   if (!s->adam_m)
     return ndq_reduce_grad_loss(s->partials, s->blocks, s->n_params, s->grad, 0, s->loss_partials, s->blocks,
@@ -494,7 +524,7 @@
                           s->best_flat, 1, stream);
   }
   ReduceTailArgs a = reduce_tail_args(*s, *s, s->partials, s->loss_partials, s->blocks, adam_step, hist_index, parity, 1,
-                                      s->best_flat);
+                                      s->best_flat, ValidArgs{}, nullptr, nullptr, nullptr, image);
   int blocks = (s->n_params + 63) / 64;
   if (oneshot) {
     ndq::Oneshot* c = static_cast<ndq::Oneshot*>(s->comm);
@@ -558,7 +588,7 @@
 }
 
 static int fit_tail(const FitCall& c, int set, bool with_train, bool with_valid, int adam_step, int hist_index, int vindex,
-                    int parity) {
+                    int parity, bool image = false) {
   const ndq_fused_fit* f = c.f;
   const ndq_fused_step& s0 = f->net[0];
   ValidArgs v{};
@@ -569,7 +599,7 @@
     const ndq_fused_step& s = f->net[k];
     a.net[k] = reduce_tail_args(s, s0, c.PART[set][k], c.LP[set], with_train ? s0.blocks : 0, with_train ? adam_step : 0,
                                 hist_index, parity, k == 0 ? 1 : 0, track ? s.best_flat : nullptr, v,
-                                set ? c.P[set][k] : nullptr, set ? c.M[set][k] : nullptr, set ? c.V[set][k] : nullptr);
+                                set ? c.P[set][k] : nullptr, set ? c.M[set][k] : nullptr, set ? c.V[set][k] : nullptr, image);
   }
   return launch_tail_multi(a, c.max_params, f->n_nets, c.max_lparts, c.stream);
 }
@@ -577,14 +607,21 @@
 static int fit_two_launch(const FitCall& c, int parity) {
   const ndq_fused_fit* f = c.f;
   const ndq_fused_step& s0 = f->net[0];
+  const bool image = f->n_nets == 1 && step_image(s0) && c.P[0][0] == s0.params;
   for (int e = 0; e < c.n_epochs; ++e, parity ^= 1) {
     if (!c.train_coords[e]) return NDQ_EINVAL;
     const bool with_valid = c.valid && e > 0;
-    int rc = f->launch(c.train_coords[e], s0.ldc, s0.n, c.P[0], c.PART[0], c.LP[0], s0.seed,
-                       with_valid ? f->valid_coords : nullptr, f->valid_ldc, with_valid ? f->valid_n : 0, c.VP[0], nullptr,
-                       c.stream);
+    int rc;
+    if (image)
+      rc = s0.launch_image(c.train_coords[e], s0.ldc, s0.n, c.P[0], c.PART[0], c.LP[0], s0.seed,
+                           with_valid ? f->valid_coords : nullptr, f->valid_ldc, with_valid ? f->valid_n : 0, c.VP[0], s0.image,
+                           s0.witness, s0.image_floats, c.stream);
+    else
+      rc = f->launch(c.train_coords[e], s0.ldc, s0.n, c.P[0], c.PART[0], c.LP[0], s0.seed,
+                     with_valid ? f->valid_coords : nullptr, f->valid_ldc, with_valid ? f->valid_n : 0, c.VP[0], nullptr,
+                     c.stream);
     if (rc) return rc;
-    rc = fit_tail(c, 0, true, with_valid, c.adam_step + e, c.hist_index + e, c.valid_index + e - 1, parity);
+    rc = fit_tail(c, 0, true, with_valid, c.adam_step + e, c.hist_index + e, c.valid_index + e - 1, parity, image);
     if (rc) return rc;
   }
   if (!c.valid) return 0;
diff --git a/neurodiffeq_amd/csrc/ndq_closure_host.h b/neurodiffeq_amd/csrc/ndq_closure_host.h
--- a/neurodiffeq_amd/csrc/ndq_closure_host.h
+++ b/neurodiffeq_amd/csrc/ndq_closure_host.h
@@ -20,14 +20,28 @@
   for (int k = 0; k < K; ++k) { a.params[k] = params[k]; a.partials[k] = partials ? partials[k] : nullptr; }
 }
 
+struct Image { const ndq::real* image; const ndq::real* witness; int floats; };
+
+template <class T> constexpr int image_floats() {
+  if constexpr (T::IMAGE) return ndq::image_supported<typename T::Cfg>() ? T::Cfg::ldsWeightsEnd(true) : 0;
+  else return 0;
+}
+template <class T> void set_image(typename T::Args& a, const Image& im) {
+  if constexpr (image_floats<T>() > 0) {
+    if (im.image && im.witness && im.floats == image_floats<T>()) { a.image = im.image; a.witness = im.witness; a.image_floats = im.floats; }
+  }
+}
+
 template <class T>
 int launch(const ndq::real* coords, int ldc, int n, const ndq::real* const* params, ndq::real* const* partials,
-           ndq::real* loss_partials, ndq::real* funcs, ndq::real* resid, int ldj, ndq::real seed, int train, void* stream) {
+           ndq::real* loss_partials, ndq::real* funcs, ndq::real* resid, int ldj, ndq::real seed, int train, void* stream,
+           const Image& im = Image{}) {
   if (!coords || !params || !loss_partials || n <= 0 || ldc < n || (train && !partials)) return -2;
   if (T::Pw::NT > 0 && !g_theta) return -2;
   typename T::Args a{};
   a.coords = coords; a.loss_partials = loss_partials;
   fill<T::K>(a, params, partials);
+  if (train) set_image<T>(a, im);
   a.funcs = funcs; a.resid = resid; a.n = n; a.ldc = ldc; a.ldj = ldj; a.seed = seed;
   a.theta = g_theta; a.theta_partials = train ? g_theta_partials : nullptr;
   hipStream_t s = static_cast<hipStream_t>(stream);
@@ -51,7 +65,7 @@
 template <class T>
 int launch_tv(const ndq::real* coords, int ldc, int n, const ndq::real* const* params, ndq::real* const* partials,
               ndq::real* loss_partials, ndq::real seed, const ndq::real* vcoords, int vldc, int vn,
-              ndq::real* vloss_partials, const void* pull, void* stream) {
+              ndq::real* vloss_partials, const void* pull, void* stream, const Image& im = Image{}) {
   if (!params || n < 0 || vn < 0 || (n == 0 && vn == 0)) return -2;
   if (n > 0 && (!coords || !partials || !loss_partials || ldc < n)) return -2;
   if (vn > 0 && (!vcoords || !vloss_partials || vldc < vn)) return -2;
@@ -59,12 +73,13 @@
   t.coords = coords; t.loss_partials = loss_partials; t.n = n; t.ldc = ldc; t.ldj = ldc; t.seed = seed;
   t.theta = g_theta; t.theta_partials = g_theta_partials;
   fill<T::K>(t, params, partials);
+  if (!pull) set_image<T>(t, im);
   v.coords = vcoords; v.loss_partials = vloss_partials; v.n = vn; v.ldc = vldc; v.ldj = vldc; v.seed = 0.f;
   v.theta = g_theta;
   fill<T::K>(v, params, nullptr);
   static const bool always_tv = getenv("NDQ_TV_ALWAYS") != nullptr;
   if (vn == 0 && !pull && !always_tv)
-    return launch<T>(coords, ldc, n, params, partials, loss_partials, nullptr, nullptr, ldc, seed, 1, stream);
+    return launch<T>(coords, ldc, n, params, partials, loss_partials, nullptr, nullptr, ldc, seed, 1, stream, im);
   const int tb = n > 0 ? fused_blocks<T>(n) : 0, vb = vn > 0 ? fused_blocks<T>(vn) : 0;
   static bool attr = false;
   if (!attr) {
@@ -138,6 +153,43 @@
 }
 #endif
 
+template <class T> int image_table(int* out) {
+  if constexpr (image_floats<T>() > 0) {
+    for (int e = 0; e < T::Cfg::P; ++e) {
+      const ndq::ImageDest d = ndq::image_dest<typename T::Cfg, true>(e);
+      out[2 * e] = d.x; out[2 * e + 1] = d.y;
+    }
+    return T::Cfg::P;
+  } else {
+    return 0;
+  }
+}
+template <class T> int image_init(const ndq::real* params, ndq::real* image, ndq::real* witness, void* stream) {
+  if constexpr (image_floats<T>() > 0) {
+    if (!params || !image || !witness) return -2;
+    const auto kern = &ndq::weight_image_init_kernel<typename T::Cfg>;
+    const int bytes = (int)sizeof(ndq::real) * image_floats<T>();
+    hipError_t e = hipFuncSetAttribute(reinterpret_cast<const void*>(kern), hipFuncAttributeMaxDynamicSharedMemorySize, bytes);
+    if (e != hipSuccess) return (int)e;
+    hipLaunchKernelGGL(kern, dim3(1), dim3(256), bytes, static_cast<hipStream_t>(stream), params, image, witness);
+    return (int)hipGetLastError();
+  } else {
+    return -2;
+  }
+}
+extern "C" int ndq_weight_image_floats() { return image_floats<Closure>(); }
+extern "C" int ndq_weight_image_table(int* out) { return out ? image_table<Closure>(out) : 0; }
+extern "C" int ndq_weight_image_init(const ndq::real* params, ndq::real* image, ndq::real* witness, void* stream) {
+  return image_init<Closure>(params, image, witness, stream);
+}
+extern "C" int ndq_weight_image_launch(const ndq::real* coords, int ldc, int n, const ndq::real* const* params,
+                                      ndq::real* const* partials, ndq::real* loss_partials, ndq::real seed,
+                                      const ndq::real* vcoords, int vldc, int vn, ndq::real* vloss_partials,
+                                      const ndq::real* image, const ndq::real* witness, int image_floats, void* stream) {
+  return launch_tv<Closure>(coords, ldc, n, params, partials, loss_partials, seed, vcoords, vldc, vn, vloss_partials, nullptr, stream,
+                            Image{image, witness, image_floats});
+}
+
 extern "C" int ndq_fused_launch(const ndq::real* coords, int ldc, int n, const ndq::real* params, ndq::real* partials,
                                 ndq::real* loss_partials, ndq::real* funcs, ndq::real* resid, int ldj, ndq::real seed,
                                 int train, void* stream) {
diff --git a/neurodiffeq_amd/csrc/ndq_mlp.h b/neurodiffeq_amd/csrc/ndq_mlp.h
--- a/neurodiffeq_amd/csrc/ndq_mlp.h
+++ b/neurodiffeq_amd/csrc/ndq_mlp.h
@@ -336,6 +336,9 @@
 #endif
 #ifndef NDQ_STAGE_INFLIGHT
 #define NDQ_STAGE_INFLIGHT 1
+#endif
+#ifndef NDQ_WEIGHT_IMAGE
+#define NDQ_WEIGHT_IMAGE 1
 #endif
 #ifndef NDQ_GROUP_PREFETCH
 #define NDQ_GROUP_PREFETCH 1
@@ -613,6 +616,44 @@
   else return v;
 }
 
+struct ImageDest { int x, y; };
+template <class C> constexpr bool image_layout() {
+  return NDQ_F64 == 0 && C::ACTP == 0 && !C::RAGGED && C::MONO == 0 && C::SKIP == 0 && C::BF16 && (C::NOUT == 1 || C::BF16O);
+}
+__host__ __device__ constexpr int frag_base(int r, int c, int ncc) {
+  return ((((r >> 4) * ncc + (c >> 5)) * 3) * 64 + (r & 15) + 16 * ((c & 15) >> 2)) * 8 + 4 * ((c & 31) >> 4) + (c & 3);
+}
+template <class C, bool BWD> __host__ __device__ constexpr ImageDest image_dest_wout(int j, int k) {
+  return ImageDest{2 * C::ldsWout(BWD) + frag_base(j, k, C::NC), BWD ? 2 * C::ldsWoutT() + frag_base(k, j, C::NCO) : -1};
+}
+template <class C, bool BWD> __host__ __device__ constexpr ImageDest image_dest(int e) {
+  constexpr int H = C::H, LS = H * H + H;
+  if (e < C::offb1) {
+    const int j = e / C::NIN, a = e - j * C::NIN;
+    return ImageDest{~(C::ldsW1T + a * H + j), -1};
+  }
+  if (e < C::offW(2)) return ImageDest{~(C::ldsb1 + (e - C::offb1)), -1};
+  if (e < C::offWout) {
+    const int l = 2 + (e - C::offW(2)) / LS, r = (e - C::offW(2)) % LS;
+    if (r >= H * H) return ImageDest{~(C::ldsb(l, BWD) + (r - H * H)), -1};
+    const int j = r / H, k = r - j * H;
+    return ImageDest{2 * C::ldsWf(l, BWD) + frag_base(j, k, C::NC), BWD ? 2 * C::ldsWt(l) + frag_base(k, j, C::NC) : -1};
+  }
+  if (e < C::offbout) {
+    if (C::NOUT == 1) return ImageDest{~(C::ldsWout(BWD) + (e - C::offWout)), -1};
+    return image_dest_wout<C, BWD>((e - C::offWout) / H, (e - C::offWout) % H);
+  }
+  return ImageDest{~(C::ldsbout(BWD) + (e - C::offbout)), -1};
+}
+__device__ __forceinline__ void image_put(real* img, const ImageDest d, real w) {
+  if (d.x < 0) { img[~d.x] = w; return; }
+  __bf16* wb = reinterpret_cast<__bf16*>(img);
+  const __bf16 w0 = (__bf16)w; const real r1 = w - (real)w0;
+  const __bf16 w1 = (__bf16)r1; const __bf16 w2 = (__bf16)(r1 - (real)w1);
+  wb[d.x] = w0; wb[d.x + 512] = w1; wb[d.x + 1024] = w2;
+  if (d.y >= 0) { wb[d.y] = w0; wb[d.y + 512] = w1; wb[d.y + 1024] = w2; }
+}
+
 template <class C, bool BWD>
 __device__ __forceinline__ void stage_weights(real* lds, const real* __restrict__ prm, int tid = -1, int nt = 0) {
   constexpr int H = C::H, D = C::D, NB = C::NB;
@@ -625,59 +666,13 @@
   };
   auto real_unit = [](int j, int hw) { return !C::RAGGED || j < hw; };
 #if NDQ_STAGE_INFLIGHT
-  if constexpr (C::ACTP == 0 && !C::RAGGED && C::MONO == 0 && C::SKIP == 0 && C::BF16 && (C::NOUT == 1 || C::BF16O)) {
-    constexpr int KP = 8, P = C::P, LS = H * H + H;
-    auto place_wout = [&](int j, int k, real w) {
-      __bf16* wf = reinterpret_cast<__bf16*>(lds + C::ldsWout(BWD));
-      __bf16* wt = reinterpret_cast<__bf16*>(lds + C::ldsWoutT());
-      const __bf16 w0 = (__bf16)w; const real r1 = w - (real)w0;
-      const __bf16 w1 = (__bf16)r1; const __bf16 w2 = (__bf16)(r1 - (real)w1);
-      {
-        const int blk = (j >> 4) * C::NC + (k >> 5);
-        const int base = ((blk * 3) * 64 + (j & 15) + 16 * ((k & 15) >> 2)) * 8 + 4 * ((k & 31) >> 4) + (k & 3);
-        wf[base] = w0; wf[base + 512] = w1; wf[base + 1024] = w2;
-      }
-      if (BWD) {
-        const int blk = (k >> 4) * C::NCO + (j >> 5);
-        const int base = ((blk * 3) * 64 + (k & 15) + 16 * ((j & 15) >> 2)) * 8 + 4 * ((j & 31) >> 4) + (j & 3);
-        wt[base] = w0; wt[base + 512] = w1; wt[base + 1024] = w2;
-      }
-    };
+  if constexpr (image_layout<C>()) {
+    constexpr int KP = 8, P = C::P;
     if constexpr (C::NOUT > 1) {
-      for (int i = C::NOUT * H + tid; i < C::HO * H; i += nt) place_wout(i / H, i % H, (real)0.f);
+      for (int i = C::NOUT * H + tid; i < C::HO * H; i += nt) image_put(lds, image_dest_wout<C, BWD>(i / H, i % H), (real)0.f);
       for (int i = C::NOUT + tid; i < C::HO; i += nt) lds[C::ldsbout(BWD) + i] = 0.f;
     }
-    auto place = [&](int e, real w) {
-      if (e < C::offb1) {
-        const int j = e / C::NIN, a = e - j * C::NIN;
-        lds[C::ldsW1T + a * H + j] = w;
-      } else if (e < C::offW(2)) {
-        lds[C::ldsb1 + (e - C::offb1)] = w;
-      } else if (e < C::offWout) {
-        const int l = 2 + (e - C::offW(2)) / LS, r = (e - C::offW(2)) % LS;
-        if (r >= H * H) { lds[C::ldsb(l, BWD) + (r - H * H)] = w; return; }
-        const int j = r / H, k = r - j * H;
-        __bf16* wf = reinterpret_cast<__bf16*>(lds + C::ldsWf(l, BWD));
-        __bf16* wt = reinterpret_cast<__bf16*>(lds + C::ldsWt(l));
-        const __bf16 w0 = (__bf16)w; const real r1 = w - (real)w0;
-        const __bf16 w1 = (__bf16)r1; const __bf16 w2 = (__bf16)(r1 - (real)w1);
-        {
-          const int blk = (j >> 4) * C::NC + (k >> 5);
-          const int base = ((blk * 3) * 64 + (j & 15) + 16 * ((k & 15) >> 2)) * 8 + 4 * ((k & 31) >> 4) + (k & 3);
-          wf[base] = w0; wf[base + 512] = w1; wf[base + 1024] = w2;
-        }
-        if (BWD) {
-          const int blk = (k >> 4) * C::NC + (j >> 5);
-          const int base = ((blk * 3) * 64 + (k & 15) + 16 * ((j & 15) >> 2)) * 8 + 4 * ((j & 31) >> 4) + (j & 3);
-          wt[base] = w0; wt[base + 512] = w1; wt[base + 1024] = w2;
-        }
-      } else if (e < C::offbout) {
-        if constexpr (C::NOUT == 1) lds[C::ldsWout(BWD) + (e - C::offWout)] = w;
-        else place_wout((e - C::offWout) / H, (e - C::offWout) % H, w);
-      } else {
-        lds[C::ldsbout(BWD) + (e - C::offbout)] = w;
-      }
-    };
+    auto place = [&](int e, real w) { image_put(lds, image_dest<C, BWD>(e), w); };
     for (int base = 0; base < P; base += KP * nt) {
       real v[KP];
 #pragma unroll
@@ -2626,6 +2621,9 @@
   real seed;
   const real* theta;
   real* theta_partials;
+  const real* image;
+  const real* witness;
+  int image_floats;
 };
 
 template <int NT>
@@ -2652,6 +2650,53 @@
 template <class C> struct no_pull_marker<C, std::void_t<decltype(C::NO_PULL)>> : std::true_type {};
 template <class C> constexpr bool pull_supported() { return NDQ_F64 == 0 && C::ACTP == 0 && !no_pull_marker<C>::value; }
 template <class C> constexpr int pull_floats() { return ((C::P + 3) & ~3) + 32; }
+
+template <class C> constexpr bool image_supported() { return NDQ_WEIGHT_IMAGE != 0 && NDQ_STAGE_INFLIGHT != 0 && image_layout<C>(); }
+template <class C, int T>
+__device__ __forceinline__ bool copy_weight_image(real* lds, const real* __restrict__ image, const real* __restrict__ prm,
+                                                  const real* __restrict__ witness) {
+  constexpr int NCH = C::ldsWeightsEnd(true) / 4, P = C::P;
+  constexpr int CPT = (NCH + T - 1) / T, EPT = (P + T - 1) / T;
+  constexpr int CB = CPT < 4 ? CPT : 4, EB = EPT < 6 ? EPT : 6;
+  constexpr int NF = (CPT + CB - 1) / CB > (EPT + EB - 1) / EB ? (CPT + CB - 1) / CB : (EPT + EB - 1) / EB;
+  const float4* img4 = reinterpret_cast<const float4*>(image);
+  float4* lds4 = reinterpret_cast<float4*>(lds);
+  const int tid = threadIdx.x;
+  bool differs = false;
+#pragma unroll 1
+  for (int f = 0; f < NF; ++f) {
+    float r[28];
+#pragma unroll
+    for (int k = 0; k < 28; ++k) r[k] = 0.f;
+#pragma unroll
+    for (int k = 0; k < CB; ++k) {
+      const int c = (f * CB + k) * T + tid;
+      const float4 v = img4[c < NCH ? c : NCH - 1];
+      r[4 * k] = v.x; r[4 * k + 1] = v.y; r[4 * k + 2] = v.z; r[4 * k + 3] = v.w;
+    }
+#pragma unroll
+    for (int k = 0; k < EB; ++k) {
+      const int e = (f * EB + k) * T + tid;
+      r[4 * CB + k] = prm[e < P ? e : P - 1];
+      r[4 * CB + EB + k] = witness[e < P ? e : P - 1];
+    }
+    asm volatile("" : "+v"(r[0]), "+v"(r[1]), "+v"(r[2]), "+v"(r[3]), "+v"(r[4]), "+v"(r[5]), "+v"(r[6]), "+v"(r[7]), "+v"(r[8]),
+                      "+v"(r[9]), "+v"(r[10]), "+v"(r[11]), "+v"(r[12]), "+v"(r[13]), "+v"(r[14]), "+v"(r[15]), "+v"(r[16]),
+                      "+v"(r[17]), "+v"(r[18]), "+v"(r[19]), "+v"(r[20]), "+v"(r[21]), "+v"(r[22]), "+v"(r[23]), "+v"(r[24]),
+                      "+v"(r[25]), "+v"(r[26]), "+v"(r[27]));
+#pragma unroll
+    for (int k = 0; k < CB; ++k) {
+      const int c = (f * CB + k) * T + tid;
+      if (c < NCH) lds4[c] = make_float4(r[4 * k], r[4 * k + 1], r[4 * k + 2], r[4 * k + 3]);
+    }
+#pragma unroll
+    for (int k = 0; k < EB; ++k) {
+      const int e = (f * EB + k) * T + tid;
+      differs |= e < P && __float_as_uint(r[4 * CB + k]) != __float_as_uint(r[4 * CB + EB + k]);
+    }
+  }
+  return differs;
+}
 
 template <class C, class PW, bool TRAIN>
 __device__ __forceinline__ void fused_closure_body(const FusedArgs& a, real* lds, const int blk, const int nblk,
@@ -2690,8 +2735,15 @@
     }
   }
 #endif
-  stage_weights<C, TRAIN>(lds, prm);
-  __syncthreads();
+  bool stage_here = true;
+  if constexpr (TRAIN && image_supported<C>()) {
+    if (a.image != nullptr && a.image_floats == C::ldsWeightsEnd(true) && prm == a.params)
+      stage_here = __syncthreads_or(copy_weight_image<C, C::BWD_THREADS>(lds, a.image, prm, a.witness) ? 1 : 0) != 0;
+  }
+  if (stage_here) {
+    stage_weights<C, TRAIN>(lds, prm);
+    __syncthreads();
+  }
   NDQ_PT(3);
   NDQ_TS(1);
   real* stage = lds + C::ldsWeightsEnd(true) + wave * C::stageFloatsPerWave;
@@ -2783,6 +2835,20 @@
   extern __shared__ __attribute__((aligned(16))) real lds[];
   const PullArgs none{};
   fused_closure_body<C, PW, TRAIN>(a, lds, blockIdx.x, gridDim.x, none, false);
+}
+
+template <class C>
+__global__ __launch_bounds__(256) void weight_image_init_kernel(const real* params, real* image, real* witness) {
+  extern __shared__ __attribute__((aligned(16))) real lds[];
+  if constexpr (image_supported<C>()) {
+    constexpr int WE = C::ldsWeightsEnd(true);
+    for (int i = threadIdx.x; i < WE; i += blockDim.x) lds[i] = 0.f;
+    __syncthreads();
+    stage_weights<C, true>(lds, params);
+    __syncthreads();
+    for (int i = threadIdx.x; i < WE; i += blockDim.x) image[i] = lds[i];
+    for (int i = threadIdx.x; i < C::P; i += blockDim.x) witness[i] = params[i];
+  }
 }
 
 template <class C, class PW>
diff --git a/neurodiffeq_amd/engine.py b/neurodiffeq_amd/engine.py
--- a/neurodiffeq_amd/engine.py
+++ b/neurodiffeq_amd/engine.py
@@ -886,6 +886,29 @@
         st.grad, st.loss_slot = fp.grad.data_ptr(), fp.grad_loss.data_ptr() + 4 * fp.numel
         st.loss_hist, st.best_loss = fs["loss_hist"].data_ptr(), fs["best_loss"].data_ptr()
 
+    def _set_image(self, st, fk):
+        if len(self.flat) != 1 or self.f64 or fk is None:
+            return
+        cache = self.__dict__.setdefault("_images", {})
+        ent = cache.get(id(fk))
+        if ent is None:
+            ent = False
+            floats, fp = fk.lib.ndq_weight_image_floats(), self.flat[0]
+            if floats > 0:
+                table = (ctypes.c_int * (2 * fp.numel))()
+                assert fk.lib.ndq_weight_image_table(table) == fp.numel
+                ent = dict(fk=fk, floats=floats, image=torch.zeros(floats, dtype=torch.float32, device=self.device),
+                           witness=torch.zeros(fp.numel, dtype=torch.float32, device=self.device),
+                           table=torch.tensor(list(table), dtype=torch.int32, device=self.device),
+                           launch=ctypes.cast(fk.lib.ndq_weight_image_launch, ctypes.c_void_p).value)
+                fp.sync()
+                _lib.check(fk.lib.ndq_weight_image_init(_ptr(fp.flat), _ptr(ent["image"]), _ptr(ent["witness"]), self._stream()),
+                           "ndq_weight_image_init")
+            cache[id(fk)] = ent
+        if ent:
+            st.launch_image, st.image_floats = ent["launch"], ent["floats"]
+            st.image, st.witness, st.image_table = ent["image"].data_ptr(), ent["witness"].data_ptr(), ent["table"].data_ptr()
+
     @staticmethod
     def _set_adam(st, m, v, group):
         st.adam_m, st.adam_v = m.data_ptr(), v.data_ptr()
@@ -958,6 +981,7 @@
             st = _lib.FusedStep()
             st.launch = b["fused_launch"]
             self._fill_step(st, 0, n, b["ld"], b["fused_blocks"], b["fused_partials"], b["fused_loss_partials"])
+            self._set_image(st, b["fusedk"])
             fs["structs"][key] = st
         n_global = n if n_global is None else n_global
         st.params = fp.flat.data_ptr()
@@ -1062,6 +1086,8 @@
                 keep.append(part)
                 self._fill_step(ff.net[k], k, *((n, ld, blocks) if K else (0, 0, 0)), part, lparts)
                 ff.net[k].best_flat = fs["best_flat"][k].data_ptr()
+            if K:
+                self._set_image(ff.net[0], fk)
             if valid is not None:
                 vparts = torch.zeros(fk.blocks(valid[1]), dtype=f32, device=dev)
                 keep.append(vparts)
```

Measured after the change: 3.047 billion collocation-points/s (median of 2 runs). About the same (-0.2%).
